# mhnazeri/PMoE

Hardware: AMD Instinct MI355X
Metric: samples/sec fwd+bwd, 256x256 RGB 4-expert PMoE (higher is better)
Workload: dtype bf16; 1 GPU; 4-expert MoE (PMoE experts), 256x256x3 x4 frames, batch 64/GPU, fwd+moe_loss+bwd, dropout 0.3; global_batch=64, parallelism=dp1

## Files before the change

pmoe_amd/csrc/conv_common.h:

```cpp
#pragma once
#include "common.h"

template <int LOG_RB, int MODE> __device__ __forceinline__ int swz_chunk(int x) {
    if (MODE == 0) return (x >> (8 - LOG_RB)) & ((1 << (LOG_RB - 4)) - 1);
    return ((x >> 1) & 1) << (LOG_RB - 5);
}

template <int LOG_RB, int MODE> __device__ __forceinline__ int lds_chunk_off(int pp, int j) {
    if (MODE == 2) return pp * 192 + (j << 4);
    return (pp << LOG_RB) + ((j ^ swz_chunk<LOG_RB, MODE>(pp)) << 4);
}

struct PatchGeom {
    int n0, n_end, e_first_img;
    int Y0, X0;
    int PH, PW, NPIX;
    int H, W, ld, coff, cmax;
    int dilate, shared;
    int step;
};

template <typename T, int LOG_RB, int NTHR, int MODE, typename TL = T>
__device__ __forceinline__ void load_halo_patch(char* patch, const T* in, const PatchGeom& g, int c0, int tid,
                                                float in_scale = 1.f) {
    constexpr int RB = 1 << LOG_RB, CPR = RB / 16, LOG_CPR = LOG_RB - 4;
    constexpr int PSTEP = NTHR / CPR;
    constexpr int VE = 16 / (int)sizeof(TL);
    constexpr bool CVT = sizeof(TL) != sizeof(T);
    constexpr int UB = CVT ? 2 : 4;
    static_assert(!CVT || (sizeof(T) == 2 && sizeof(TL) == 1), "conversion on load: bf16 -> fp8 only");
    const int pj = tid & (CPR - 1);
    int pp = tid >> LOG_CPR;
    int ix = pp % g.PW;
    const int row = pp / g.PW;
    int iy = row % g.PH, pn = row / g.PH;
    while (pp < g.NPIX) {
        v4i v[UB], v2[CVT ? UB : 1];
        int dst[UB];
#pragma unroll
        for (int u = 0; u < UB; ++u) {
            dst[u] = -1;
            if (pp < g.NPIX) {
                const int n = g.n0 + pn;
                int Y = g.Y0 + iy * g.step, X = g.X0 + ix * g.step;
                bool ok = n < g.n_end && (c0 + pj * VE) < g.cmax;
                if (g.dilate) {
                    ok = ok && Y >= 0 && X >= 0 && !((Y | X) & 1);
                    Y >>= 1; X >>= 1;
                    ok = ok && Y < g.H && X < g.W;
                } else {
                    ok = ok && (unsigned)Y < (unsigned)g.H && (unsigned)X < (unsigned)g.W;
                }
                v[u] = v4i{0, 0, 0, 0};
                if (CVT) v2[u] = v4i{0, 0, 0, 0};
                if (ok) {
                    const int nin = g.shared ? (n - g.e_first_img) : n;
                    const T* src = in + (((size_t)nin * g.H + Y) * g.W + X) * g.ld + g.coff + c0 + pj * VE;
                    v[u] = ldg16(src);
                    if (CVT) v2[u] = ldg16(src + 8);
                }
                dst[u] = pp * RB + ((pj ^ swz_chunk<LOG_RB, MODE>(pp)) << 4);
                pp += PSTEP;
                ix += PSTEP;
                while (ix >= g.PW) {
                    ix -= g.PW;
                    if (++iy == g.PH) { iy = 0; ++pn; }
                }
            }
        }
#pragma unroll
        for (int u = 0; u < UB; ++u)
            if (dst[u] >= 0) {
                if (CVT) *reinterpret_cast<v4i*>(patch + dst[u]) = cvt16_bf16_to_fp8(v[u], v2[u], in_scale);
                else *reinterpret_cast<v4i*>(patch + dst[u]) = v[u];
            }
    }
}

template <typename T, int LOG_RB, int NTHR, int MAXV>
struct PatchStage {
    static constexpr int RB = 1 << LOG_RB, CPR = RB / 16, LOG_CPR = LOG_RB - 4;
    static constexpr int PSTEP = NTHR / CPR;
    static constexpr int VE = 16 / (int)sizeof(T);
    v4i v[MAXV];

    __device__ __forceinline__ void issue(const T* in, const PatchGeom& g, int c0, int tid) {
        const int pj = tid & (CPR - 1);
        int pp = tid >> LOG_CPR;
        int ix = pp % g.PW;
        const int row = pp / g.PW;
        int iy = row % g.PH, pn = row / g.PH;
        const bool cok = (c0 + pj * VE) < g.cmax;
#pragma unroll
        for (int u = 0; u < MAXV; ++u) {
            v[u] = v4i{0, 0, 0, 0};
            if (pp < g.NPIX) {
                const int n = g.n0 + pn;
                int Y = g.Y0 + iy * g.step, X = g.X0 + ix * g.step;
                bool ok = cok && n < g.n_end;
                if (g.dilate) {
                    ok = ok && Y >= 0 && X >= 0 && !((Y | X) & 1);
                    Y >>= 1; X >>= 1;
                    ok = ok && Y < g.H && X < g.W;
                } else {
                    ok = ok && (unsigned)Y < (unsigned)g.H && (unsigned)X < (unsigned)g.W;
                }
                if (ok) {
                    const int nin = g.shared ? (n - g.e_first_img) : n;
                    v[u] = ldg16(in + (((size_t)nin * g.H + Y) * g.W + X) * g.ld + g.coff + c0 + pj * VE);
                }
            }
            pp += PSTEP;
            ix += PSTEP;
            while (ix >= g.PW) {
                ix -= g.PW;
                if (++iy == g.PH) { iy = 0; ++pn; }
            }
        }
    }

    template <int MODE> __device__ __forceinline__ void commit(char* patch, int npix, int tid) const {
        const int pj = tid & (CPR - 1);
#pragma unroll
        for (int u = 0; u < MAXV; ++u) {
            const int pp = (tid >> LOG_CPR) + u * PSTEP;
            if (pp < npix) *reinterpret_cast<v4i*>(patch + lds_chunk_off<LOG_RB, MODE>(pp, pj)) = v[u];
        }
    }
};
```

pmoe_amd/csrc/conv_dma.hip:

```cpp
#include "conv_common.h"
#include <stdlib.h>
#include "kernels.h"

namespace {

constexpr int RB = 128, LOG_RB = 7, CK = 64, BM = 256, BN = 128, NTHR = 512, VE = 8;
constexpr int WSLOT = BN * RB;
constexpr int RING = 4;
typedef __attribute__((address_space(3))) void lds_void;

__device__ __forceinline__ int cswz(int x) { return (x >> 1) & 7; }

#define VMCNT(n) asm volatile("s_waitcnt vmcnt(" #n ")" ::: "memory")

#ifdef PMOE_STAMP
#define STAMP_INIT unsigned long long st_prev = __builtin_amdgcn_s_memtime(); const unsigned long long st_r0 = __builtin_amdgcn_s_memrealtime(); unsigned st_acc[4] = {0, 0, 0, 0};
#define LAP(i) { const unsigned long long st_t = __builtin_amdgcn_s_memtime(); st_acc[i] += (unsigned)(st_t - st_prev); st_prev = st_t; }
#else
#define STAMP_INIT
#define LAP(i)
#endif

#define VMCASE(n) case n: VMCNT(n); break;
__device__ __forceinline__ void vm_wait_prod(int n) {
    switch (n) {
        VMCASE(0) VMCASE(1) VMCASE(2) VMCASE(3) VMCASE(4) VMCASE(5) VMCASE(6) VMCASE(7) VMCASE(8) VMCASE(9) VMCASE(10) VMCASE(11)
        VMCASE(12) VMCASE(13) VMCASE(14) VMCASE(15) VMCASE(16) VMCASE(17) VMCASE(18) VMCASE(19) VMCASE(20) VMCASE(21) VMCASE(22)
        VMCASE(23)
        default: VMCNT(24); break;
    }
}

template <bool MF16, bool PROD = false>
__global__ void __launch_bounds__(PROD ? NTHR + 64 : NTHR, PROD ? 1 : 2) conv3x3_dma_kernel(const ConvArgs a_in, const int pbuf_bytes) {
    ConvArgs a = a_in;
    if constexpr (PROD) {
        a.res_mode = PMOE_RES_NONE; a.res = nullptr;
        a.bias = nullptr; a.act = PMOE_ACT_NONE; a.drop_p = 0.f; a.bn = nullptr;
    }
    extern __shared__ __attribute__((aligned(16))) char smem[];
    STAMP_INIT
    const int tid = threadIdx.x, lane = tid & 63;
    const int wave = __builtin_amdgcn_readfirstlane(tid >> 6);
    const int l31 = lane & 31, h = lane >> 5;
    const int wm = wave >> 1, wn = wave & 1;

    const int nblk = a.CoutP / BN;
    const unsigned flat = xcd_remap(blockIdx.x, gridDim.x);
    const unsigned mb = flat / nblk;
    const int nb = (int)(flat % nblk);
    int t = (int)mb;
    const int px_t = t % a.tiles_x; t /= a.tiles_x;
    const int py_t = t % a.tiles_y; t /= a.tiles_y;
    const int ng = t % a.n_groups;
    const int e = t / a.n_groups;
    const int lTW = a.lTW, lTH = a.lTH;
    const int TW = 1 << lTW, TH = 1 << lTH;
    const int PW = TW + 2, PH = TH + 2;
    const int NPIX = a.TN * PH * PW;
    const int NPIECE = (NPIX + 7) >> 3;
    const int n0 = e * a.ipe + ng * a.TN, n_end = (e + 1) * a.ipe;
    const int oy0 = py_t * TH, ox0 = px_t * TW;
    const int cout0 = nb * BN;

    char* wring = smem + 2 * pbuf_bytes;

    const bf16* inb = (const bf16*)a.in + (size_t)n0 * a.H * a.W * a.in_ld + a.in_coff;
    long long in_bytes = ((long long)(n_end - n0) * a.H * a.W * a.in_ld - a.in_coff) * 2;
    if (in_bytes > 0x7ff00000ll) in_bytes = 0x7ff00000ll;
    const __amdgpu_buffer_rsrc_t rs_in = __builtin_amdgcn_make_buffer_rsrc((void*)inb, (short)0, (int)in_bytes, 0x00020000);
    const bf16* wb = (const bf16*)a.w + ((size_t)e * a.CoutP + cout0) * 9 * a.Cin;
    const __amdgpu_buffer_rsrc_t rs_w = __builtin_amdgcn_make_buffer_rsrc((void*)wb, (short)0, BN * 9 * a.Cin * 2, 0x00020000);

    constexpr int OOB = 0x7ff80000;
    if constexpr (PROD) {
        if (wave == 8) {
            int pv[48], wv[16];
#pragma unroll
            for (int i = 0; i < 48; ++i) {
                const int pp = (i << 3) + (lane >> 3);
                const int jj = lane & 7;
                const int px = pp % PW;
                const int rowq = pp / PW;
                const int prow = rowq % PH, pn = rowq / PH;
                const int Y = oy0 - 1 + prow, X = ox0 - 1 + px;
                const bool ok = pp < NPIX && n0 + pn < n_end && (unsigned)Y < (unsigned)a.H && (unsigned)X < (unsigned)a.W;
                pv[i] = ok ? ((((pn * a.H + Y) * a.W + X) * a.in_ld) << 1) + ((jj ^ cswz(px)) << 4) : OOB;
            }
#pragma unroll
            for (int i = 0; i < 16; ++i) {
                const int row = (i << 3) + (lane >> 3);
                wv[i] = ((row * 9 * a.Cin) << 1) + (((lane & 7) ^ cswz(row)) << 4);
            }
            auto req_w = [&](int slot, int tap, int c0) {
#pragma unroll
                for (int i = 0; i < 16; ++i)
                    __builtin_amdgcn_raw_ptr_buffer_load_lds(rs_w, (lds_void*)(wring + slot * WSLOT + (i << 10)), 16, wv[i],
                                                             (tap * a.Cin + c0) << 1, 0, 0);
            };
            const int nch = a.Cin / CK, TT = nch * 9;
            int after = 0;
            for (int ch = 0; ch < nch; ++ch) {
                const int c0 = ch * CK;
                const bool more = ch + 1 < nch;
#pragma unroll
                for (int tap = 0; tap < 9; ++tap) {
                    const int tt = ch * 9 + tap;
                    vm_wait_prod(after);
                    __builtin_amdgcn_s_barrier();
                    int n = 0;
                    if (tap >= 1 && tap <= 6 && more) {
#pragma unroll
                        for (int j = 0; j < 8; ++j) {
                            const int idx = (tap - 1) * 8 + j;
                            if (idx < NPIECE) {
                                __builtin_amdgcn_raw_ptr_buffer_load_lds(
                                    rs_in, (lds_void*)(smem + ((ch + 1) & 1) * pbuf_bytes + (idx << 10)), 16, pv[idx], (c0 + CK) << 1, 0, 0);
                                ++n;
                            }
                        }
                    }
                    if (tt + 2 < TT) {
                        int ntap = tap + 2, nc0 = c0;
                        if (ntap >= 9) { ntap -= 9; nc0 += CK; }
                        req_w((tt + 2) & (RING - 1), ntap, nc0);
                        n += 16;
                    }
                    after = n;
                }
            }
            return;
        }
    }
    int pvoff[6];
#pragma unroll
    for (int i = 0; i < 6; ++i) {
        const int pp = ((wave + 8 * i) << 3) + (lane >> 3);
        const int jj = lane & 7;
        int px = pp % PW;
        const int rowq = pp / PW;
        const int prow = rowq % PH, pn = rowq / PH;
        const int Y = oy0 - 1 + prow, X = ox0 - 1 + px;
        const bool ok = pp < NPIX && n0 + pn < n_end && (unsigned)Y < (unsigned)a.H && (unsigned)X < (unsigned)a.W;
        pvoff[i] = ok ? ((((pn * a.H + Y) * a.W + X) * a.in_ld) << 1) + ((jj ^ cswz(px)) << 4) : OOB;
    }
    int wvoff[2];
#pragma unroll
    for (int i = 0; i < 2; ++i) {
        const int row = ((wave + 8 * i) << 3) + (lane >> 3);
        wvoff[i] = ((row * 9 * a.Cin) << 1) + (((lane & 7) ^ cswz(row)) << 4);
    }
    const int my_pieces = (NPIECE - wave + 7) >> 3;

    auto dma_patch = [&](int i, int buf, int c0) {
        __builtin_amdgcn_raw_ptr_buffer_load_lds(rs_in, (lds_void*)(smem + buf * pbuf_bytes + ((wave + 8 * i) << 10)), 16,
                                                 pvoff[i], c0 << 1, 0, 0);
    };
    auto dma_w = [&](int slot, int tap, int c0) {
#pragma unroll
        for (int i = 0; i < 2; ++i)
            __builtin_amdgcn_raw_ptr_buffer_load_lds(rs_w, (lds_void*)(wring + slot * WSLOT + ((wave + 8 * i) << 10)), 16,
                                                     wvoff[i], (tap * a.Cin + c0) << 1, 0, 0);
    };

    int pbase[2], pcol[2];
#pragma unroll
    for (int mt = 0; mt < 2; ++mt) {
        const int p = wm * 64 + mt * 32 + l31;
        const int mx = p & (TW - 1), my = (p >> lTW) & (TH - 1), pn = p >> (lTW + lTH);
        pbase[mt] = ((pn * PH + my) * PW + mx) << LOG_RB;
        pcol[mt] = mx;
    }
    int aoff[2][4];
#pragma unroll
    for (int nt = 0; nt < 2; ++nt)
#pragma unroll
        for (int ks = 0; ks < 4; ++ks) {
            const int row = wn * 64 + nt * 32 + l31;
            aoff[nt][ks] = row * RB + (((ks * 2 + h) ^ cswz(row)) << 4);
        }

    f32x16 acc[2][2];
#pragma unroll
    for (int i = 0; i < 2; ++i)
#pragma unroll
        for (int j = 0; j < 2; ++j)
#pragma unroll
            for (int k = 0; k < 16; ++k) acc[i][j][k] = 0.f;
    f32x4 acc16[4][4];
    int pbase16[4], pcol16[4], aoff16[4][2];
    if constexpr (MF16) {
#pragma unroll
        for (int i = 0; i < 4; ++i)
#pragma unroll
            for (int j = 0; j < 4; ++j) acc16[i][j] = f32x4{0.f, 0.f, 0.f, 0.f};
#pragma unroll
        for (int mt = 0; mt < 4; ++mt) {
            const int p = wm * 64 + mt * 16 + (lane & 15);
            const int mx = p & (TW - 1), my = (p >> lTW) & (TH - 1), pn = p >> (lTW + lTH);
            pbase16[mt] = ((pn * PH + my) * PW + mx) << LOG_RB;
            pcol16[mt] = mx;
        }
#pragma unroll
        for (int nt = 0; nt < 4; ++nt)
#pragma unroll
            for (int ks = 0; ks < 2; ++ks) {
                const int row = wn * 64 + nt * 16 + (lane & 15);
                aoff16[nt][ks] = row * RB + (((ks * 4 + (lane >> 4)) ^ cswz(row)) << 4);
            }
    }

    const int nchunks = a.Cin / CK;
    const int T = nchunks * 9;

    const bool zpre_on = !PROD && (a.res_mode == PMOE_RES_DBN || a.res_mode == PMOE_RES_ADD) && !a.bias && a.act == PMOE_ACT_NONE &&
                         a.drop_p == 0.f;
    v4i zpre[8];
#pragma unroll
    for (int u = 0; u < 8; ++u) zpre[u] = v4i{0, 0, 0, 0};

#pragma unroll
    for (int i = 0; i < 6; ++i)
        if (i < my_pieces) dma_patch(i, 0, 0);
    dma_w(0, 0, 0);
    dma_w(1, 1, 0);

    for (int ch = 0; ch < nchunks; ++ch) {
        const int c0 = ch * CK;
        const char* patch = smem + (ch & 1) * pbuf_bytes;
        const bool more = ch + 1 < nchunks;
#pragma unroll
        for (int tap = 0; tap < 9; ++tap) {
            const int tt = ch * 9 + tap;
            const bool prev_piece = tap >= 2 && tap <= 7 && more && (tap - 2) < my_pieces;
            if constexpr (PROD) {
                if (tt == 0) VMCNT(0);
            } else {
                if (tt + 1 >= T) VMCNT(0);
                else if (zpre_on && !more && tap == 1) VMCNT(10);
                else if (prev_piece) VMCNT(3);
                else VMCNT(2);
            }
            __builtin_amdgcn_s_barrier();
#ifdef PMOE_STAMP
            if (tt == 0) LAP(0)
#endif
            if constexpr (!PROD) {
            if (tap >= 1 && tap <= 6 && more && (tap - 1) < my_pieces) dma_patch(tap - 1, (ch + 1) & 1, c0 + CK);
            if (tt + 2 < T) {
                int ntap = tap + 2, nc0 = c0;
                if (ntap >= 9) { ntap -= 9; nc0 += CK; }
                dma_w((tt + 2) & (RING - 1), ntap, nc0);
            }
            }
            if (tap == 0 && zpre_on && !more) {
                const int zc = tid & 15, zr = tid >> 4;
#pragma unroll
                for (int u = 0; u < 8; ++u) {
                    const int p = zr + u * 32;
                    const int mx = p & (TW - 1), my = (p >> lTW) & (TH - 1), pn = p >> (lTW + lTH);
                    const int n = n0 + pn, oy = oy0 + my, ox = ox0 + mx;
                    const bool ok = cout0 + zc * VE < a.Cout && n < n_end && oy < a.Ho && ox < a.Wo;
                    const size_t off = ok ? (((size_t)n * a.Ho + oy) * a.Wo + ox) * a.res_ld + a.res_coff + cout0 + zc * VE : (size_t)0;
                    zpre[u] = ldg16((const bf16*)a.res + off);
                }
            }
            const char* wt = wring + (tt & (RING - 1)) * WSLOT;
            const int tapoff = ((tap / 3) * PW + (tap % 3)) << LOG_RB;
            if constexpr (MF16) {
                int bsw16[4];
                const char* bp16[4];
#pragma unroll
                for (int mt = 0; mt < 4; ++mt) {
                    bp16[mt] = patch + pbase16[mt] + tapoff;
                    bsw16[mt] = cswz(pcol16[mt] + (tap % 3));
                }
#pragma unroll
                for (int ks = 0; ks < 2; ++ks) {
                    v4i af[4], bfr[4];
#pragma unroll
                    for (int nt = 0; nt < 4; ++nt) af[nt] = *reinterpret_cast<const v4i*>(wt + aoff16[nt][ks]);
#pragma unroll
                    for (int mt = 0; mt < 4; ++mt)
                        bfr[mt] = *reinterpret_cast<const v4i*>(bp16[mt] + (((ks * 4 + (lane >> 4)) ^ bsw16[mt]) << 4));
#pragma unroll
                    for (int nt = 0; nt < 4; ++nt)
#pragma unroll
                        for (int mt = 0; mt < 4; ++mt)
                            acc16[nt][mt] = __builtin_amdgcn_mfma_f32_16x16x32_bf16(__builtin_bit_cast(bf16x8, af[nt]),
                                                                                    __builtin_bit_cast(bf16x8, bfr[mt]),
                                                                                    acc16[nt][mt], 0, 0, 0);
                }
                continue;
            }
            int bsw[2];
            const char* bp[2];
#pragma unroll
            for (int mt = 0; mt < 2; ++mt) {
                bp[mt] = patch + pbase[mt] + tapoff;
                bsw[mt] = cswz(pcol[mt] + (tap % 3));
            }
#pragma unroll
            for (int ks = 0; ks < 4; ++ks) {
                v4i af[2], bfr[2];
#pragma unroll
                for (int nt = 0; nt < 2; ++nt) af[nt] = *reinterpret_cast<const v4i*>(wt + aoff[nt][ks]);
#pragma unroll
                for (int mt = 0; mt < 2; ++mt)
                    bfr[mt] = *reinterpret_cast<const v4i*>(bp[mt] + (((ks * 2 + h) ^ bsw[mt]) << 4));
#pragma unroll
                for (int nt = 0; nt < 2; ++nt)
#pragma unroll
                    for (int mt = 0; mt < 2; ++mt)
                        acc[nt][mt] = __builtin_amdgcn_mfma_f32_32x32x16_bf16(__builtin_bit_cast(bf16x8, af[nt]),
                                                                              __builtin_bit_cast(bf16x8, bfr[mt]),
                                                                              acc[nt][mt], 0, 0, 0);
            }
        }
    }

#define DMA_ZPRE zpre
#define DMA_ZPRE_ON zpre_on
#define DMA_HAS_MF16
#include "conv_dma_epilogue.inc"
#undef DMA_ZPRE
#undef DMA_ZPRE_ON
#undef DMA_HAS_MF16
}

template <bool MF16, bool NARROW = false>
__global__ void __launch_bounds__(NTHR + 4 * 64, 1) conv3x3_dma_stream_kernel(const ConvArgs a_in, const int pbuf_bytes, const int ntiles,
                                                                          const int magic_pw, const int magic_ph) {
    constexpr int NT = NARROW ? 1 : 2, WPC = 4 * NT;
    static_assert(!(NARROW && MF16), "the 64-cout tile exists on the 32x32x16 shape only");
    constexpr int BN = 64 * NT, WSLOT = BN * RB;
    STAMP_INIT
    ConvArgs a = a_in;
    a.res_mode = PMOE_RES_NONE; a.res = nullptr; a.bias = nullptr; a.act = PMOE_ACT_NONE; a.drop_p = 0.f; a.bn = nullptr;
    extern __shared__ __attribute__((aligned(16))) char smem[];
    const int tid = threadIdx.x, lane = tid & 63;
    const int wave = __builtin_amdgcn_readfirstlane(tid >> 6);
    const int l31 = lane & 31, h = lane >> 5;
    const int wm = (wave >> 1) & 3, wn = wave & 1;
    const int nblk = a.CoutP / BN;
    const int lTW = a.lTW, lTH = a.lTH;
    const int TW = 1 << lTW, TH = 1 << lTH;
    const int PW = TW + 2, PH = TH + 2;
    const int NPIX = a.TN * PH * PW;
    const int NPIECE = (NPIX + 7) >> 3;
    char* wring = smem + 2 * pbuf_bytes;
    const int nchunks = a.Cin / CK;
    const int T = nchunks * 9;
    const int G = (int)gridDim.x;
    const int b0 = (int)xcd_remap(blockIdx.x, gridDim.x);
    const int nbar_epi = a.stats ? 4 : 2;
    struct Tile { int e, n0, n_end, oy0, ox0, cout0; unsigned mb; };
    auto decode = [&](int L) {
        Tile q;
        q.mb = (unsigned)(L / nblk);
        const int nb = L % nblk;
        int t = (int)q.mb;
        const int px_t = t % a.tiles_x; t /= a.tiles_x;
        const int py_t = t % a.tiles_y; t /= a.tiles_y;
        const int ng = t % a.n_groups;
        q.e = t / a.n_groups;
        q.n0 = q.e * a.ipe + ng * a.TN; q.n_end = (q.e + 1) * a.ipe;
        q.oy0 = py_t * TH; q.ox0 = px_t * TW; q.cout0 = nb * BN;
        return q;
    };
    constexpr int OOB = 0x7ff80000;

    if (wave >= 8) {
        const int pw = wave - 8;
        auto rs_in_of = [&](const Tile& q) {
            const bf16* inb = (const bf16*)a.in + (size_t)q.e * a.ipe * a.H * a.W * a.in_ld + a.in_coff;
            return __builtin_amdgcn_make_buffer_rsrc((void*)inb, (short)0, (int)(((long long)a.ipe * a.H * a.W * a.in_ld - a.in_coff) * 2),
                                                     0x00020000);
        };
        auto rs_w_of = [&](const Tile& q) {
            const bf16* wb = (const bf16*)a.w + ((size_t)q.e * a.CoutP + q.cout0) * 9 * a.Cin;
            return __builtin_amdgcn_make_buffer_rsrc((void*)wb, (short)0, BN * 9 * a.Cin * 2, 0x00020000);
        };
        int L = b0;
        if (L >= ntiles) return;
        int gtt = 0, gch = 0;
        if (pw >= 2) {
            const int pp2 = pw - 2;
            const int lrow = lane >> 3, ljj = lane & 7;
            auto req_patch = [&](const Tile& q, const __amdgpu_buffer_rsrc_t& rs, int i, int buf, int c0, int opaque) {
                const int pp = (i << 3) + lrow + opaque;
                const int rowq = (pp * magic_pw) >> 16, px = pp - rowq * PW;
                const int pn = (rowq * magic_ph) >> 16, prow = rowq - pn * PH;
                const int n = q.n0 - q.e * a.ipe + pn, Y = q.oy0 - 1 + prow, X = q.ox0 - 1 + px;
                const bool ok = pp < NPIX && n < a.ipe && (unsigned)Y < (unsigned)a.H && (unsigned)X < (unsigned)a.W;
                const int off = ((((n * a.H + Y) * a.W + X) * a.in_ld) << 1) + ((ljj ^ cswz(px)) << 4);
                __builtin_amdgcn_raw_ptr_buffer_load_lds(rs, (lds_void*)(smem + buf * pbuf_bytes + (i << 10)), 16, ok ? off : OOB, c0 << 1, 0, 0);
            };
            Tile cur = decode(L);
            __amdgpu_buffer_rsrc_t rin = rs_in_of(cur);
            for (int i = pp2; i < NPIECE; i += 2) req_patch(cur, rin, i, 0, 0, 0);
            int after = 0;
            for (;;) {
                const bool has_next = L + G < ntiles;
                const Tile nxt = decode(has_next ? L + G : L);
                const __amdgpu_buffer_rsrc_t rin_n = rs_in_of(nxt);
                for (int ch = 0; ch < nchunks; ++ch) {
                    const int c0 = ch * CK;
                    const bool more = ch + 1 < nchunks;
                    int opaque = 0;
                    asm volatile("" : "+s"(opaque));
#pragma unroll
                    for (int tap = 0; tap < 9; ++tap) {
                        vm_wait_prod(after);
                        __builtin_amdgcn_s_barrier();
                        int n = 0;
                        if (tap >= 1 && tap <= 6 && (more || has_next)) {
#pragma unroll
                            for (int j = 0; j < 4; ++j) {
                                const int idx = (tap - 1) * 8 + 2 * j + pp2;
                                if (idx < NPIECE) {
                                    if (more) req_patch(cur, rin, idx, (gch + ch + 1) & 1, c0 + CK, opaque);
                                    else req_patch(nxt, rin_n, idx, (gch + ch + 1) & 1, 0, opaque);
                                    ++n;
                                }
                            }
                        }
                        after = n;
                    }
                }
                for (int i = 0; i < nbar_epi; ++i) __builtin_amdgcn_s_barrier();
                if (!has_next) return;
                gch += nchunks;
                L += G; cur = nxt; rin = rin_n;
            }
        }
        int wv[8];
#pragma unroll
        for (int i = 0; i < WPC; ++i) {
            const int row = ((2 * i + pw) << 3) + (lane >> 3);
            wv[i] = ((row * 9 * a.Cin) << 1) + (((lane & 7) ^ cswz(row)) << 4);
        }
        auto req_w = [&](const __amdgpu_buffer_rsrc_t& rs, int slot, int tap, int c0) {
#pragma unroll
            for (int i = 0; i < WPC; ++i)
                __builtin_amdgcn_raw_ptr_buffer_load_lds(rs, (lds_void*)(wring + slot * WSLOT + ((2 * i + pw) << 10)), 16, wv[i],
                                                         (tap * a.Cin + c0) << 1, 0, 0);
        };
        Tile cur = decode(L);
        __amdgpu_buffer_rsrc_t rw = rs_w_of(cur);
        req_w(rw, 0, 0, 0);
        req_w(rw, 1, 1, 0);
        int after = WPC;
        for (;;) {
            const bool has_next = L + G < ntiles;
            const Tile nxt = decode(has_next ? L + G : L);
            const __amdgpu_buffer_rsrc_t rw_n = rs_w_of(nxt);
            for (int ch = 0; ch < nchunks; ++ch) {
                const int c0 = ch * CK;
#pragma unroll
                for (int tap = 0; tap < 9; ++tap) {
                    const int tt = ch * 9 + tap;
                    vm_wait_prod(after);
                    __builtin_amdgcn_s_barrier();
                    int n = 0;
                    if (tt + 2 < T) {
                        int ntap = tap + 2, nc0 = c0;
                        if (ntap >= 9) { ntap -= 9; nc0 += CK; }
                        req_w(rw, (gtt + tt + 2) & (RING - 1), ntap, nc0);
                        n = WPC;
                    } else if (has_next) {
                        req_w(rw_n, (gtt + tt + 2) & (RING - 1), tt + 2 - T, 0);
                        n = WPC;
                    }
                    after = n;
                }
            }
            for (int i = 0; i < nbar_epi; ++i) __builtin_amdgcn_s_barrier();
            if (!has_next) return;
            gtt += T;
            L += G; cur = nxt; rw = rw_n;
        }
    }

    int pbase[2], pcol[2];
#pragma unroll
    for (int mt = 0; mt < 2; ++mt) {
        const int p = wm * 64 + mt * 32 + l31;
        const int mx = p & (TW - 1), my = (p >> lTW) & (TH - 1), pn = p >> (lTW + lTH);
        pbase[mt] = ((pn * PH + my) * PW + mx) << LOG_RB;
        pcol[mt] = mx;
    }
    int aoff[NT][4];
#pragma unroll
    for (int nt = 0; nt < NT; ++nt)
#pragma unroll
        for (int ks = 0; ks < 4; ++ks) {
            const int row = wn * (32 * NT) + nt * 32 + l31;
            aoff[nt][ks] = row * RB + (((ks * 2 + h) ^ cswz(row)) << 4);
        }
    int pbase16[4], pcol16[4], aoff16[4][2];
    if constexpr (MF16) {
#pragma unroll
        for (int mt = 0; mt < 4; ++mt) {
            const int p = wm * 64 + mt * 16 + (lane & 15);
            const int mx = p & (TW - 1), my = (p >> lTW) & (TH - 1), pn = p >> (lTW + lTH);
            pbase16[mt] = ((pn * PH + my) * PW + mx) << LOG_RB;
            pcol16[mt] = mx;
        }
#pragma unroll
        for (int nt = 0; nt < 4; ++nt)
#pragma unroll
            for (int ks = 0; ks < 2; ++ks) {
                const int row = wn * 64 + nt * 16 + (lane & 15);
                aoff16[nt][ks] = row * RB + (((ks * 4 + (lane >> 4)) ^ cswz(row)) << 4);
            }
    }
    int gtt = 0, gch = 0;
    for (int L = b0; L < ntiles; L += G) {
        const Tile q = decode(L);
        const int e = q.e, n0 = q.n0, n_end = q.n_end, oy0 = q.oy0, ox0 = q.ox0, cout0 = q.cout0;
        const unsigned mb = q.mb;
        f32x16 acc[NT][2];
        f32x4 acc16[4][4];
        if constexpr (MF16) {
#pragma unroll
            for (int i = 0; i < 4; ++i)
#pragma unroll
                for (int j = 0; j < 4; ++j) acc16[i][j] = f32x4{0.f, 0.f, 0.f, 0.f};
        } else {
#pragma unroll
            for (int i = 0; i < NT; ++i)
#pragma unroll
                for (int j = 0; j < 2; ++j)
#pragma unroll
                    for (int k = 0; k < 16; ++k) acc[i][j][k] = 0.f;
        }
        for (int ch = 0; ch < nchunks; ++ch) {
            const char* patch = smem + ((gch + ch) & 1) * pbuf_bytes;
#pragma unroll
            for (int tap = 0; tap < 9; ++tap) {
                const int tt = ch * 9 + tap;
                __builtin_amdgcn_s_barrier();
                const char* wt = wring + ((gtt + tt) & (RING - 1)) * WSLOT;
                const int tapoff = ((tap / 3) * PW + (tap % 3)) << LOG_RB;
                if constexpr (MF16) {
                    int bsw16[4];
                    const char* bp16[4];
#pragma unroll
                    for (int mt = 0; mt < 4; ++mt) {
                        bp16[mt] = patch + pbase16[mt] + tapoff;
                        bsw16[mt] = cswz(pcol16[mt] + (tap % 3));
                    }
#pragma unroll
                    for (int ks = 0; ks < 2; ++ks) {
                        v4i af[4], bfr[4];
#pragma unroll
                        for (int nt = 0; nt < 4; ++nt) af[nt] = *reinterpret_cast<const v4i*>(wt + aoff16[nt][ks]);
#pragma unroll
                        for (int mt = 0; mt < 4; ++mt)
                            bfr[mt] = *reinterpret_cast<const v4i*>(bp16[mt] + (((ks * 4 + (lane >> 4)) ^ bsw16[mt]) << 4));
#pragma unroll
                        for (int nt = 0; nt < 4; ++nt)
#pragma unroll
                            for (int mt = 0; mt < 4; ++mt)
                                acc16[nt][mt] = __builtin_amdgcn_mfma_f32_16x16x32_bf16(__builtin_bit_cast(bf16x8, af[nt]),
                                                                                        __builtin_bit_cast(bf16x8, bfr[mt]),
                                                                                        acc16[nt][mt], 0, 0, 0);
                    }
                } else {
                    int bsw[2];
                    const char* bp[2];
#pragma unroll
                    for (int mt = 0; mt < 2; ++mt) {
                        bp[mt] = patch + pbase[mt] + tapoff;
                        bsw[mt] = cswz(pcol[mt] + (tap % 3));
                    }
#pragma unroll
                    for (int ks = 0; ks < 4; ++ks) {
                        v4i af[NT], bfr[2];
#pragma unroll
                        for (int nt = 0; nt < NT; ++nt) af[nt] = *reinterpret_cast<const v4i*>(wt + aoff[nt][ks]);
#pragma unroll
                        for (int mt = 0; mt < 2; ++mt)
                            bfr[mt] = *reinterpret_cast<const v4i*>(bp[mt] + (((ks * 2 + h) ^ bsw[mt]) << 4));
#pragma unroll
                        for (int nt = 0; nt < NT; ++nt)
#pragma unroll
                            for (int mt = 0; mt < 2; ++mt)
                                acc[nt][mt] = __builtin_amdgcn_mfma_f32_32x32x16_bf16(__builtin_bit_cast(bf16x8, af[nt]),
                                                                                      __builtin_bit_cast(bf16x8, bfr[mt]),
                                                                                      acc[nt][mt], 0, 0, 0);
                    }
                }
            }
        }
        gtt += T; gch += nchunks;
        char* stg_lo = smem + ((gch - 1) & 1) * pbuf_bytes;
        char* stg_s0 = wring + ((gtt + 2) & (RING - 1)) * WSLOT;
        char* stg_s1 = wring + ((gtt + 3) & (RING - 1)) * WSLOT;
#define DMA_STG_ROW(p) (NT == 1 ? stg_lo + (p) * 128 : (p) < 160 ? stg_lo + (p) * 256 : (p) < 224 ? stg_s0 + ((p) - 160) * 256 : stg_s1 + ((p) - 224) * 256)
#define DMA_RED_BASE stg_lo
#define DMA_HAS_MF16
#define DMA_NT NT
#include "conv_dma_epilogue.inc"
#undef DMA_STG_ROW
#undef DMA_RED_BASE
#undef DMA_HAS_MF16
#undef DMA_NT
    }
}

__device__ __forceinline__ void vm_wait_upto(int n) {
    switch (n) {
        case 0: VMCNT(0); break; case 1: VMCNT(1); break; case 2: VMCNT(2); break; case 3: VMCNT(3); break;
        case 4: VMCNT(4); break; case 5: VMCNT(5); break; case 6: VMCNT(6); break; case 7: VMCNT(7); break;
        case 8: VMCNT(8); break; case 9: VMCNT(9); break; case 10: VMCNT(10); break; case 11: VMCNT(11); break;
        case 12: VMCNT(12); break; case 13: VMCNT(13); break; case 14: VMCNT(14); break; case 15: VMCNT(15); break;
        default: VMCNT(16); break;
    }
}

constexpr int RING3 = 3;

template <bool CLS>
__global__ void __launch_bounds__(NTHR, 2) conv3x3s2_dma_kernel(const ConvArgs a, const int pbuf_bytes) {
    extern __shared__ __attribute__((aligned(16))) char smem[];
    STAMP_INIT
    const int tid = threadIdx.x, lane = tid & 63;
    const int wave = __builtin_amdgcn_readfirstlane(tid >> 6);
    const int l31 = lane & 31, h = lane >> 5;
    const int wm = wave >> 1, wn = wave & 1;

    const int nblk = (a.CoutP + BN - 1) / BN;
    const unsigned flat = xcd_remap(blockIdx.x, gridDim.x);
    const unsigned mb = flat / nblk;
    const int nb = (int)(flat % nblk);
    int t = (int)mb;
    const int px_t = t % a.tiles_x; t /= a.tiles_x;
    const int py_t = t % a.tiles_y; t /= a.tiles_y;
    const int ng = t % a.n_groups;
    const int e = t / a.n_groups;
    const int lTW = a.lTW, lTH = a.lTH;
    const int TW = 1 << lTW, TH = 1 << lTH;
    const int PW = TW + 1, PH = TH + 1;
    const int NPIX = a.TN * PH * PW;
    const int NPIECE = (NPIX + 7) >> 3;
    const int n0 = e * a.ipe + ng * a.TN, n_end = (e + 1) * a.ipe;
    const int oy0 = py_t * TH, ox0 = px_t * TW;
    const int cout0 = nb * BN;

    char* wring = smem + 3 * pbuf_bytes;

    const bf16* inb = (const bf16*)a.in + (size_t)n0 * a.H * a.W * a.in_ld + a.in_coff;
    long long in_bytes = ((long long)(n_end - n0) * a.H * a.W * a.in_ld - a.in_coff) * 2;
    if (in_bytes > 0x7ff00000ll) in_bytes = 0x7ff00000ll;
    const __amdgpu_buffer_rsrc_t rs_in = __builtin_amdgcn_make_buffer_rsrc((void*)inb, (short)0, (int)in_bytes, 0x00020000);
    const bf16* wb = (const bf16*)a.w + ((size_t)e * a.CoutP + cout0) * 9 * a.Cin;
    const int wrows = a.CoutP - cout0 < BN ? a.CoutP - cout0 : BN;
    const __amdgpu_buffer_rsrc_t rs_w = __builtin_amdgcn_make_buffer_rsrc((void*)wb, (short)0, wrows * 9 * a.Cin * 2, 0x00020000);

    constexpr int OOB = 0x7ff80000;
    int pvoff[6];
    unsigned vbits = 0;
#pragma unroll
    for (int i = 0; i < 6; ++i) {
        const int pp = ((wave + 8 * i) << 3) + (lane >> 3);
        const int jj = lane & 7;
        const int bx = pp % PW;
        const int rowq = pp / PW;
        const int by = rowq % PH, pn = rowq / PH;
        if constexpr (CLS) {
            const int By = oy0 + by, Bx = ox0 + bx;
            const bool ok = pp < NPIX && n0 + pn < n_end && By < a.H && Bx < a.W;
            pvoff[i] = ok ? ((((pn * a.H + By) * a.W + Bx) * a.in_ld) << 1) + ((jj ^ cswz(bx)) << 4) : OOB;
        } else {
        const int By = oy0 - 1 + by, Bx = ox0 - 1 + bx;
        const bool okb = pp < NPIX && n0 + pn < n_end && By >= 0 && Bx >= 0;
        pvoff[i] = okb ? ((((pn * a.H + 2 * By) * a.W + 2 * Bx) * a.in_ld) << 1) + ((jj ^ cswz(bx)) << 4) : OOB;
        const unsigned vb = (okb && 2 * By < a.H ? 1u : 0u) | (okb && 2 * By + 1 < a.H ? 2u : 0u) |
                            (2 * Bx < a.W ? 4u : 0u) | (2 * Bx + 1 < a.W ? 8u : 0u);
        vbits |= vb << (4 * i);
        }
    }
    int wvoff[2];
#pragma unroll
    for (int i = 0; i < 2; ++i) {
        const int row = ((wave + 8 * i) << 3) + (lane >> 3);
        wvoff[i] = ((row * 9 * a.Cin) << 1) + (((lane & 7) ^ cswz(row)) << 4);
    }
    const int my_pieces = (NPIECE - wave + 7) >> 3;

    auto dma_patch = [&](int buf, int pl, int c0) {
        const int py = pl < 2, px = (pl & 1) == 0;
        const int soff = (c0 << 1) + (CLS ? 0 : (((py * a.W + px) * a.in_ld) << 1));
#pragma unroll
        for (int i = 0; i < 6; ++i)
            if (i < my_pieces) {
                const bool ok = CLS || (((vbits >> (4 * i + py)) & 1u) && ((vbits >> (4 * i + 2 + px)) & 1u));
                __builtin_amdgcn_raw_ptr_buffer_load_lds(rs_in, (lds_void*)(smem + buf * pbuf_bytes + ((wave + 8 * i) << 10)), 16,
                                                         ok ? pvoff[i] : OOB, soff, 0, 0);
            }
    };
    auto dma_w = [&](int slot, int tap, int c0) {
#pragma unroll
        for (int i = 0; i < 2; ++i)
            __builtin_amdgcn_raw_ptr_buffer_load_lds(rs_w, (lds_void*)(wring + slot * WSLOT + ((wave + 8 * i) << 10)), 16,
                                                     wvoff[i], (tap * a.Cin + c0) << 1, 0, 0);
    };
    auto tap_of = [&](int pl, int tp, int& ktap, int& oy, int& ox) {
        if constexpr (CLS) {
            oy = a.kw == 2 ? (tp >> 1) : tp; ox = a.kw == 2 ? (tp & 1) : 0;
            ktap = tp == 0 ? a.tapmap[0] : tp == 1 ? a.tapmap[1] : tp == 2 ? a.tapmap[2] : a.tapmap[3];
            return;
        }
        const int py = pl < 2, px = (pl & 1) == 0;
        const int iy = px ? (tp >> 1) : tp, ix = px ? (tp & 1) : 0;
        const int ky = py ? 2 * iy : 1, kx = px ? 2 * ix : 1;
        ktap = ky * 3 + kx;
        oy = ky != 0; ox = kx != 0;
    };
    auto ntaps = [&](int pl) { return CLS ? a.kh * a.kw : pl == 0 ? 4 : pl == 3 ? 1 : 2; };

    int pbase[2], pcol[2];
#pragma unroll
    for (int mt = 0; mt < 2; ++mt) {
        const int p = wm * 64 + mt * 32 + l31;
        const int mx = p & (TW - 1), my = (p >> lTW) & (TH - 1), pn = p >> (lTW + lTH);
        pbase[mt] = ((pn * PH + my) * PW + mx) << LOG_RB;
        pcol[mt] = mx;
    }
    int aoff[2][4];
#pragma unroll
    for (int nt = 0; nt < 2; ++nt)
#pragma unroll
        for (int ks = 0; ks < 4; ++ks) {
            const int row = wn * 64 + nt * 32 + l31;
            aoff[nt][ks] = row * RB + (((ks * 2 + h) ^ cswz(row)) << 4);
        }

    f32x16 acc[2][2];
#pragma unroll
    for (int i = 0; i < 2; ++i)
#pragma unroll
        for (int j = 0; j < 2; ++j)
#pragma unroll
            for (int k = 0; k < 16; ++k) acc[i][j][k] = 0.f;

    const int nch = a.Cin / CK;
    const int T = CLS ? nch * a.kh * a.kw : nch * 9, NSTEP = CLS ? nch : nch * 4;

    int c1 = 0, p1 = 0, p2 = 0;
    int len1 = 0, len2 = 0;
    auto step_plane = [&](int s) { return CLS ? 0 : s / nch; };
    auto step_c0 = [&](int s) { return (s % nch) * CK; };
    int pl2 = 0, ch2 = 0, tp2 = 0;
    auto advance2 = [&]() {
        if (++tp2 == ntaps(pl2)) { tp2 = 0; if (++ch2 == nch) { ch2 = 0; ++pl2; } }
    };

    dma_patch(0, step_plane(0), step_c0(0));
    if (NSTEP > 1) dma_patch(1, step_plane(1), step_c0(1));
    {
        int kt, oy, ox;
        tap_of(pl2, tp2, kt, oy, ox); dma_w(0, kt, ch2 * CK); advance2();
        if (T > 1) { tap_of(pl2, tp2, kt, oy, ox); dma_w(1, kt, ch2 * CK); advance2(); c1 = 2; }
    }

    int tt = 0, wslot = 0;
    for (int s = 0, sbuf = 0; s < NSTEP; ++s, sbuf = sbuf == 2 ? 0 : sbuf + 1) {
        const int pl = step_plane(s);
        const char* patch = smem + sbuf * pbuf_bytes;
        const int nt_s = ntaps(pl);
        for (int tp = 0; tp < nt_s; ++tp, ++tt, wslot = wslot == 2 ? 0 : wslot + 1) {
            const bool patch_last = tp == 0 && s >= 2 && len1 == 1 && len2 == 1;
            vm_wait_upto(c1 + (patch_last ? 0 : p2));
            __builtin_amdgcn_s_barrier();
            int cnow = 0, pnow = 0;
            if (tt + 2 < T) {
                int kt, oy2, ox2;
                tap_of(pl2, tp2, kt, oy2, ox2);
                dma_w(wslot == 0 ? 2 : wslot - 1, kt, ch2 * CK);
                cnow = 2;
                advance2();
            }
            if (tp == 0 && s + 2 < NSTEP) {
                dma_patch(sbuf == 0 ? 2 : sbuf - 1, step_plane(s + 2), step_c0(s + 2));
                pnow = my_pieces;
            }
            c1 = cnow + pnow; p2 = p1; p1 = pnow;
            int ktap, oy, ox;
            tap_of(pl, tp, ktap, oy, ox);
            const char* wt = wring + wslot * WSLOT;
            const int tapoff = (oy * PW + ox) << LOG_RB;
            int bsw[2];
            const char* bp[2];
#pragma unroll
            for (int mt = 0; mt < 2; ++mt) {
                bp[mt] = patch + pbase[mt] + tapoff;
                bsw[mt] = cswz(pcol[mt] + ox);
            }
#pragma unroll
            for (int ks = 0; ks < 4; ++ks) {
                v4i af[2], bfr[2];
#pragma unroll
                for (int nt = 0; nt < 2; ++nt) af[nt] = *reinterpret_cast<const v4i*>(wt + aoff[nt][ks]);
#pragma unroll
                for (int mt = 0; mt < 2; ++mt)
                    bfr[mt] = *reinterpret_cast<const v4i*>(bp[mt] + (((ks * 2 + h) ^ bsw[mt]) << 4));
#pragma unroll
                for (int nt = 0; nt < 2; ++nt)
#pragma unroll
                    for (int mt = 0; mt < 2; ++mt)
                        acc[nt][mt] = __builtin_amdgcn_mfma_f32_32x32x16_bf16(__builtin_bit_cast(bf16x8, af[nt]),
                                                                              __builtin_bit_cast(bf16x8, bfr[mt]),
                                                                              acc[nt][mt], 0, 0, 0);
            }
        }
        len2 = len1; len1 = nt_s;
    }

    if constexpr (CLS) {
#define DMA_LATTICE
#include "conv_dma_epilogue.inc"
#undef DMA_LATTICE
    } else {
#include "conv_dma_epilogue.inc"
    }
}

typedef int v8i __attribute__((ext_vector_type(8)));

__global__ void __launch_bounds__(NTHR, 2) conv3x3_dma_f8_kernel(const ConvArgs a, const int pbuf_bytes) {
    extern __shared__ __attribute__((aligned(16))) char smem[];
    STAMP_INIT
    constexpr int CK8 = 128;
    const int tid = threadIdx.x, lane = tid & 63;
    const int wave = __builtin_amdgcn_readfirstlane(tid >> 6);
    const int l31 = lane & 31, h = lane >> 5;
    const int wm = wave >> 1, wn = wave & 1;

    const int nblk = a.CoutP / BN;
    const unsigned flat = xcd_remap(blockIdx.x, gridDim.x);
    const unsigned mb = flat / nblk;
    const int nb = (int)(flat % nblk);
    int t = (int)mb;
    const int px_t = t % a.tiles_x; t /= a.tiles_x;
    const int py_t = t % a.tiles_y; t /= a.tiles_y;
    const int ng = t % a.n_groups;
    const int e = t / a.n_groups;
    const int lTW = a.lTW, lTH = a.lTH;
    const int TW = 1 << lTW, TH = 1 << lTH;
    const int PW = TW + 2, PH = TH + 2;
    const int NPIX = a.TN * PH * PW;
    const int NPIECE = (NPIX + 7) >> 3;
    const int n0 = e * a.ipe + ng * a.TN, n_end = (e + 1) * a.ipe;
    const int oy0 = py_t * TH, ox0 = px_t * TW;
    const int cout0 = nb * BN;

    char* wring = smem + 2 * pbuf_bytes;

    const unsigned char* inb = (const unsigned char*)a.in + (size_t)n0 * a.H * a.W * a.in_ld + a.in_coff;
    long long in_bytes = (long long)(n_end - n0) * a.H * a.W * a.in_ld - a.in_coff;
    if (in_bytes > 0x7ff00000ll) in_bytes = 0x7ff00000ll;
    const __amdgpu_buffer_rsrc_t rs_in = __builtin_amdgcn_make_buffer_rsrc((void*)inb, (short)0, (int)in_bytes, 0x00020000);
    const unsigned char* wb = (const unsigned char*)a.w + ((size_t)e * a.CoutP + cout0) * 9 * a.Cin;
    const __amdgpu_buffer_rsrc_t rs_w = __builtin_amdgcn_make_buffer_rsrc((void*)wb, (short)0, BN * 9 * a.Cin, 0x00020000);

    constexpr int OOB = 0x7ff80000;
    int pvoff[6];
#pragma unroll
    for (int i = 0; i < 6; ++i) {
        const int pp = ((wave + 8 * i) << 3) + (lane >> 3);
        const int jj = lane & 7;
        int px = pp % PW;
        const int rowq = pp / PW;
        const int prow = rowq % PH, pn = rowq / PH;
        const int Y = oy0 - 1 + prow, X = ox0 - 1 + px;
        const bool ok = pp < NPIX && n0 + pn < n_end && (unsigned)Y < (unsigned)a.H && (unsigned)X < (unsigned)a.W;
        pvoff[i] = ok ? (((pn * a.H + Y) * a.W + X) * a.in_ld) + ((jj ^ cswz(px)) << 4) : OOB;
    }
    int wvoff[2];
#pragma unroll
    for (int i = 0; i < 2; ++i) {
        const int row = ((wave + 8 * i) << 3) + (lane >> 3);
        wvoff[i] = (row * 9 * a.Cin) + (((lane & 7) ^ cswz(row)) << 4);
    }
    const int my_pieces = (NPIECE - wave + 7) >> 3;

    auto dma_patch = [&](int i, int buf, int c0) {
        __builtin_amdgcn_raw_ptr_buffer_load_lds(rs_in, (lds_void*)(smem + buf * pbuf_bytes + ((wave + 8 * i) << 10)), 16,
                                                 pvoff[i], c0, 0, 0);
    };
    auto dma_w = [&](int slot, int tap, int c0) {
#pragma unroll
        for (int i = 0; i < 2; ++i)
            __builtin_amdgcn_raw_ptr_buffer_load_lds(rs_w, (lds_void*)(wring + slot * WSLOT + ((wave + 8 * i) << 10)), 16,
                                                     wvoff[i], tap * a.Cin + c0, 0, 0);
    };

    int pbase[2], pcol[2];
#pragma unroll
    for (int mt = 0; mt < 2; ++mt) {
        const int p = wm * 64 + mt * 32 + l31;
        const int mx = p & (TW - 1), my = (p >> lTW) & (TH - 1), pn = p >> (lTW + lTH);
        pbase[mt] = ((pn * PH + my) * PW + mx) << LOG_RB;
        pcol[mt] = mx;
    }
    int arow[2], asw[2];
#pragma unroll
    for (int nt = 0; nt < 2; ++nt) {
        const int row = wn * 64 + nt * 32 + l31;
        arow[nt] = row * RB;
        asw[nt] = cswz(row);
    }

    f32x16 acc[2][2];
#pragma unroll
    for (int i = 0; i < 2; ++i)
#pragma unroll
        for (int j = 0; j < 2; ++j)
#pragma unroll
            for (int k = 0; k < 16; ++k) acc[i][j][k] = 0.f;

    const int nchunks = a.Cin / CK8;
    const int T = nchunks * 9;

#pragma unroll
    for (int i = 0; i < 6; ++i)
        if (i < my_pieces) dma_patch(i, 0, 0);
    dma_w(0, 0, 0);
    dma_w(1, 1, 0);

    for (int ch = 0; ch < nchunks; ++ch) {
        const int c0 = ch * CK8;
        const char* patch = smem + (ch & 1) * pbuf_bytes;
        const bool more = ch + 1 < nchunks;
#pragma unroll 1
        for (int tap = 0; tap < 9; ++tap) {
            const int tt = ch * 9 + tap;
            const bool prev_piece = tap >= 2 && tap <= 7 && more && (tap - 2) < my_pieces;
            if (tt + 1 >= T) VMCNT(0);
            else if (prev_piece) VMCNT(3);
            else VMCNT(2);
            __builtin_amdgcn_s_barrier();
            if (tap >= 1 && tap <= 6 && more && (tap - 1) < my_pieces) dma_patch(tap - 1, (ch + 1) & 1, c0 + CK8);
            if (tt + 2 < T) {
                int ntap = tap + 2, nc0 = c0;
                if (ntap >= 9) { ntap -= 9; nc0 += CK8; }
                dma_w((tt + 2) & (RING - 1), ntap, nc0);
            }
            const char* wt = wring + (tt & (RING - 1)) * WSLOT;
            const int tapoff = ((tap / 3) * PW + (tap % 3)) << LOG_RB;
            int bsw[2];
            const char* bp[2];
#pragma unroll
            for (int mt = 0; mt < 2; ++mt) {
                bp[mt] = patch + pbase[mt] + tapoff;
                bsw[mt] = cswz(pcol[mt] + (tap % 3));
            }
#pragma unroll
            for (int ks = 0; ks < 2; ++ks) {
                v8i af[2], bfr[2];
#pragma unroll
                for (int nt = 0; nt < 2; ++nt) {
                    const v4i lo = *reinterpret_cast<const v4i*>(wt + arow[nt] + (((ks * 4 + 2 * h) ^ asw[nt]) << 4));
                    const v4i hi = *reinterpret_cast<const v4i*>(wt + arow[nt] + (((ks * 4 + 2 * h + 1) ^ asw[nt]) << 4));
                    af[nt] = v8i{lo[0], lo[1], lo[2], lo[3], hi[0], hi[1], hi[2], hi[3]};
                }
#pragma unroll
                for (int mt = 0; mt < 2; ++mt) {
                    const v4i lo = *reinterpret_cast<const v4i*>(bp[mt] + (((ks * 4 + 2 * h) ^ bsw[mt]) << 4));
                    const v4i hi = *reinterpret_cast<const v4i*>(bp[mt] + (((ks * 4 + 2 * h + 1) ^ bsw[mt]) << 4));
                    bfr[mt] = v8i{lo[0], lo[1], lo[2], lo[3], hi[0], hi[1], hi[2], hi[3]};
                }
#pragma unroll
                for (int nt = 0; nt < 2; ++nt)
#pragma unroll
                    for (int mt = 0; mt < 2; ++mt)
                        acc[nt][mt] = __builtin_amdgcn_mfma_scale_f32_32x32x64_f8f6f4(af[nt], bfr[mt], acc[nt][mt], 0, 0, 0, 0x7f, 0, 0x7f);
            }
        }
    }

#define DMA_OSCALE
#include "conv_dma_epilogue.inc"
#undef DMA_OSCALE
}

}

static bool dma_tile(const ConvArgs& a, int halo, int ltw_max, int nbuf, int ring, int esz, ConvLaunch* l) {
    if ((long long)a.ipe * a.Ho * a.Wo < 4096) return false;
    auto p2 = [](int v) { int l = 0; while ((1 << l) < v) ++l; return l; };
    int lTW = p2(a.Wo); if (lTW > ltw_max) lTW = ltw_max;
    if (lTW < 4) return false;
    int lTH = p2(a.Ho); if (lTH > 8 - lTW) lTH = 8 - lTW;
    const int TN = BM >> (lTW + lTH);
    const int npiece = (TN * ((1 << lTH) + halo) * ((1 << lTW) + halo) + 7) / 8;
    if (npiece > 48) return false;
    const int pb = npiece * 1024;
    const size_t need = (size_t)nbuf * pb + (size_t)ring * WSLOT;
    if (need > 160 * 1024) return false;
    if ((long long)a.ipe * a.H * a.W * a.in_ld * esz >= 0x7ff00000ll) return false;
    ConvArgs& c = l->a;
    c = a;
    c.lTW = lTW; c.lTH = lTH; c.TN = TN;
    c.n_groups = (a.ipe + TN - 1) / TN;
    c.tiles_y = (a.Ho + (1 << lTH) - 1) >> lTH;
    c.tiles_x = (a.Wo + (1 << lTW) - 1) >> lTW;
    l->mblocks = (a.N / a.ipe) * c.n_groups * c.tiles_y * c.tiles_x;
    l->smem = need < (size_t)BM / 2 * BN * 4 ? (size_t)BM / 2 * BN * 4 : need;
    l->pbuf = pb;
    return true;
}

bool conv_dma_plan(const ConvArgs& a, int dtype, ConvLaunch* l) {
    const char* ev = getenv("PMOE_CONV_DMA");
    if ((ev && !atoi(ev)) || dtype != PMOE_DT_BF16 || a.w_fp8) return false;
    if (a.ks != 3 || a.kh != 3 || a.kw != 3 || a.use_tapmap || a.stride != 1 || a.pad != 1 || a.dilate || a.in_shared) return false;
    if (a.out_step != 1 || a.Ho != a.H || a.Wo != a.W) return false;
    if (a.Cin % CK || a.Cout % 8 || a.N % a.ipe) return false;
    const bool plain = a.res_mode == PMOE_RES_NONE && !a.bias && a.act == PMOE_ACT_NONE && a.drop_p == 0.f;
    const char* evn = getenv("PMOE_DMA_NARROW");
    bool narrow = !(evn && !atoi(evn)) && a.CoutP == 64 && a.Cin >= 2 * CK && plain;
    const char* evs = getenv("PMOE_DMA_STREAM");
    bool stream = !(evs && !atoi(evs)) && plain && (a.Cin <= 256 || (evs && atoi(evs) == 2));
#ifdef PMOE_STAMP
    narrow = stream = false;
#endif
    if (a.CoutP % BN && !narrow) return false;
    if (!dma_tile(a, 2, 5, 2, RING, 2, l)) return false;
    const ConvArgs& c = l->a;
    const int PW = (1 << c.lTW) + 2, PH = (1 << c.lTH) + 2;
    const int npiece = (c.TN * PH * PW + 7) / 8;
    const bool stream_ok = l->pbuf >= 160 * 256 && magic_div_exact(npiece * 8, PW, PH, &l->mpw, &l->mph) &&
                           c.TN * PH < 1024 && PW < 1024 && a.ipe < 2047;
    if (narrow && !stream_ok) return false;
    const char* evm = getenv("PMOE_DMA_MF16");
    const char* evp = getenv("PMOE_DMA_PRODUCER");
    l->kind = CONV_DMA;
    l->narrow = narrow;
    l->stream = narrow || (stream && stream_ok);
    l->producer = !l->stream && !(evp && !atoi(evp)) && plain && (a.Cin >= 256 || (evp && atoi(evp) == 2));
    l->mf16 = !narrow && (evm ? atoi(evm) != 0 : a.Cin >= 256);
    l->code = narrow ? 5067 : (l->mf16 ? 5017 : 5007) + (l->stream ? 40 : l->producer ? 20 : 0);
    return true;
}

bool conv_dma_s2_plan(const ConvArgs& a, int dtype, ConvLaunch* l) {
    const char* ev = getenv("PMOE_CONV_S2DMA");
    if ((ev && !atoi(ev)) || dtype != PMOE_DT_BF16 || a.w_fp8) return false;
    if (a.ks != 3 || a.kh != 3 || a.kw != 3 || a.use_tapmap || a.stride != 2 || a.pad != 1 || a.dilate || a.in_shared) return false;
    if (a.out_step != 1 || a.Ho != (a.H - 1) / 2 + 1 || a.Wo != (a.W - 1) / 2 + 1) return false;
    if (a.Cin % CK || a.CoutP % BN || a.Cout % 8 || a.N % a.ipe) return false;
    if (a.res_mode == PMOE_RES_DBN) return false;
    if (!dma_tile(a, 1, 4, 3, RING3, 2, l)) return false;
    l->kind = CONV_DMA_S2;
    l->code = 5207;
    return true;
}

bool conv_dma_s2cls_plan(const ConvArgs& a, int dtype, ConvLaunch* l) {
    const char* ev = getenv("PMOE_CONV_S2DMA");
    if ((ev && !atoi(ev)) || dtype != PMOE_DT_BF16 || a.w_fp8) return false;
    if (a.ks != 3 || !a.use_tapmap || a.out_step != 2 || a.stride != 1 || a.pad != 0 || a.dilate || a.in_shared) return false;
    if (a.kh < 1 || a.kh > 2 || a.kw < 1 || a.kw > 2) return false;
    const char* e64 = getenv("PMOE_S2CLS_64");
    if (a.Cin % CK || a.CoutP % ((e64 && atoi(e64)) ? 64 : BN) || a.Cout % 8 || a.N % a.ipe || a.stats || a.res_mode > PMOE_RES_ADD) return false;
    if (!dma_tile(a, 1, 4, 3, RING3, 2, l)) return false;
    l->kind = CONV_DMA_S2CLS;
    l->code = 5207;
    return true;
}

bool conv_dma_f8_plan(const ConvArgs& a, int dtype, ConvLaunch* l) {
    const char* ev = getenv("PMOE_CONV_F8DMA");
    if ((ev && !atoi(ev)) || dtype != PMOE_DT_BF16 || !a.w_fp8 || !a.in_fp8 || !a.oscale) return false;
    if (a.ks != 3 || a.kh != 3 || a.kw != 3 || a.use_tapmap || a.stride != 1 || a.pad != 1 || a.dilate || a.in_shared) return false;
    if (a.out_step != 1 || a.Ho != a.H || a.Wo != a.W || a.res_mode != PMOE_RES_NONE) return false;
    if (a.Cin % 128 || a.CoutP % BN || a.Cout % 8 || a.N % a.ipe || a.in_ld % 16 || a.in_coff % 16) return false;
    if (!dma_tile(a, 2, 5, 2, RING, 1, l)) return false;
    l->kind = CONV_DMA_F8;
    l->code = 8507;
    return true;
}

template <auto KERNEL, typename... Args> static int dma_go(dim3 grid, int nthr, size_t smem, hipStream_t st, Args... args) {
    HIP_RET((ensure_dyn_lds<KERNEL>(160 * 1024)));
    hipLaunchKernelGGL(KERNEL, grid, dim3(nthr), smem, st, args...);
    return (int)hipGetLastError();
}

int conv_dma_launch(const ConvLaunch& l, hipStream_t st) {
    const ConvArgs& a = l.a;
    const int wgs = l.mblocks * (a.CoutP / BN);
    switch (l.kind) {
    case CONV_DMA_F8: return dma_go<conv3x3_dma_f8_kernel>(dim3(wgs), NTHR, l.smem, st, a, l.pbuf);
    case CONV_DMA_S2: return dma_go<conv3x3s2_dma_kernel<false>>(dim3(wgs), NTHR, l.smem, st, a, l.pbuf);
    case CONV_DMA_S2CLS:
        return dma_go<conv3x3s2_dma_kernel<true>>(dim3(l.mblocks * ((a.CoutP + BN - 1) / BN)), NTHR, l.smem, st, a, l.pbuf);
    case CONV_DMA: break;
    default: return PMOE_ERR_ARG;
    }
    if (l.stream) {
        const int ntiles = l.narrow ? l.mblocks : wgs;
        const dim3 grid(ntiles < 256 ? ntiles : 256);
        if (l.narrow) return dma_go<conv3x3_dma_stream_kernel<false, true>>(grid, NTHR + 4 * 64, l.smem, st, a, l.pbuf, ntiles, l.mpw, l.mph);
        if (l.mf16) return dma_go<conv3x3_dma_stream_kernel<true>>(grid, NTHR + 4 * 64, l.smem, st, a, l.pbuf, ntiles, l.mpw, l.mph);
        return dma_go<conv3x3_dma_stream_kernel<false>>(grid, NTHR + 4 * 64, l.smem, st, a, l.pbuf, ntiles, l.mpw, l.mph);
    }
    if (l.producer) {
        if (l.mf16) return dma_go<conv3x3_dma_kernel<true, true>>(dim3(wgs), NTHR + 64, l.smem, st, a, l.pbuf);
        return dma_go<conv3x3_dma_kernel<false, true>>(dim3(wgs), NTHR + 64, l.smem, st, a, l.pbuf);
    }
    if (l.mf16) return dma_go<conv3x3_dma_kernel<true>>(dim3(wgs), NTHR, l.smem, st, a, l.pbuf);
    return dma_go<conv3x3_dma_kernel<false>>(dim3(wgs), NTHR, l.smem, st, a, l.pbuf);
}
```

pmoe_amd/csrc/conv_wgrad.hip:

```cpp
#include "conv_common.h"
#include <stdlib.h>
#include "kernels.h"

template <typename T> struct WgradCfg;
template <> struct WgradCfg<bf16> { static constexpr int WCO = 2, WCI = 2, WK = 2, NW = 8; };
template <> struct WgradCfg<float> { static constexpr int WCO = 1, WCI = 1, WK = 4, NW = 4; };

typedef __attribute__((address_space(3))) s16x4 lds_s16x4;

__device__ __forceinline__ s16x4 tr_read(const char* p) {
    return __builtin_amdgcn_ds_read_tr16_b64_v4i16((lds_s16x4*)(p));
}

template <typename T, int TAPS, int MAXV>
__global__ void __launch_bounds__(WgradCfg<T>::NW * 64) conv_wgrad_kernel(const WgradArgs a) {
    constexpr int NTHR = WgradCfg<T>::NW * 64;
    constexpr int LOG_RB = 7, RB = 128;
    constexpr int VE = 16 / (int)sizeof(T);
    constexpr int CKW = RB / (int)sizeof(T);
    constexpr int WCI = WgradCfg<T>::WCI, WK = WgradCfg<T>::WK;
    constexpr int KS = TAPS == 9 ? 3 : 1;
    constexpr int MAXDY = 256 * 8 / NTHR;
    extern __shared__ __attribute__((aligned(16))) char smem[];

    const int tid = threadIdx.x, lane = tid & 63, wave = tid >> 6;
    const int l31 = lane & 31, h = lane >> 5;
    constexpr int WCO = WgradCfg<T>::WCO;
    const int ci_sub = wave % WCI;
    const int co_sub = (wave / WCI) % WCO;
    const int k_sub = wave / (WCI * WCO);

    const int e = blockIdx.z;
    const int n_ci_blk = (a.Cin + CKW - 1) / CKW;
    const int npairs = n_ci_blk * ((a.Cout + CKW - 1) / CKW);
    const unsigned flat = xcd_remap(blockIdx.x, gridDim.x);
    const int nsplit = (int)(gridDim.x / npairs);
    const int pair = a.slice_fastest ? (int)(blockIdx.x / nsplit) : (int)(flat % npairs);
    const int split = a.slice_fastest ? (int)(blockIdx.x % nsplit) : (int)(flat / npairs);
    const int cob = pair / n_ci_blk, cib = pair % n_ci_blk;
    const int co0 = cob * CKW, ci0 = cib * CKW;

    const int lTW = a.lTW, lTH = a.lTH;
    const int TW = 1 << lTW, TH = 1 << lTH;
    const int S = KS == 1 ? 1 : a.stride, step = KS == 1 ? a.stride : 1;
    const int PW = (TW - 1) * S + KS, PH = (TH - 1) * S + KS;
    const int NPIX = a.TN * PH * PW;
    const int BMP = a.TN << (lTW + lTH);
    const int mbpe = a.n_groups * a.tiles_y * a.tiles_x;

    char* dyt = smem;
    constexpr int RS = 192;
    char* patch = smem + BMP * RS;

    f32x16 acc[TAPS];
#pragma unroll
    for (int t = 0; t < TAPS; ++t)
#pragma unroll
        for (int k = 0; k < 16; ++k) acc[t][k] = 0.f;

    const T* x = (const T*)a.x;
    const T* dy = (const T*)a.dy;
    const int mb_begin = split * a.mb_per_wg;
    int mb_end = mb_begin + a.mb_per_wg;
    if (mb_end > mbpe) mb_end = mbpe;

    PatchStage<T, LOG_RB, NTHR, MAXV> xs;
    v4i dyv[MAXDY];
    const int dyj = tid & 7;
    const bool dy_cok = co0 + dyj * VE < a.Cout;

    auto issue = [&](int mbi) {
        int t = mbi;
        const int px = t % a.tiles_x; t /= a.tiles_x;
        const int py = t % a.tiles_y; t /= a.tiles_y;
        const int ng = t;
        const int n0 = e * a.ipe + ng * a.TN, n_end = (e + 1) * a.ipe;
        const int oy0 = py * TH, ox0 = px * TW;
#pragma unroll
        for (int u = 0; u < MAXDY; ++u) {
            const int p = (tid >> 3) + u * (NTHR / 8);
            const int mx = p & (TW - 1), my = (p >> lTW) & (TH - 1), pn = p >> (lTW + lTH);
            const int n = n0 + pn, oy = oy0 + my, ox = ox0 + mx;
            dyv[u] = v4i{0, 0, 0, 0};
            if (p < BMP && dy_cok && n < n_end && oy < a.Ho && ox < a.Wo)
                dyv[u] = ldg16(dy + (((size_t)n * a.Ho + oy) * a.Wo + ox) * a.dy_ld + a.dy_coff + co0 + dyj * VE);
        }
        PatchGeom geo;
        geo.n0 = n0; geo.n_end = n_end; geo.e_first_img = e * a.ipe;
        geo.Y0 = oy0 * a.stride - a.pad; geo.X0 = ox0 * a.stride - a.pad; geo.PH = PH; geo.PW = PW; geo.NPIX = NPIX;
        geo.H = a.H; geo.W = a.W; geo.ld = a.x_ld; geo.coff = a.x_coff; geo.cmax = a.Cin;
        geo.dilate = 0; geo.shared = a.x_shared; geo.step = step;
        xs.issue(x, geo, ci0, tid);
    };
    auto commit = [&]() {
#pragma unroll
        for (int u = 0; u < MAXDY; ++u) {
            const int p = (tid >> 3) + u * (NTHR / 8);
            if (p < BMP) *reinterpret_cast<v4i*>(dyt + lds_chunk_off<LOG_RB, 2>(p, dyj)) = dyv[u];
        }
        xs.template commit<2>(patch, NPIX, tid);
    };

    if (mb_begin < mb_end) issue(mb_begin);
    for (int mbi = mb_begin; mbi < mb_end; ++mbi) {
        __syncthreads();
        commit();
        __syncthreads();
        if (mbi + 1 < mb_end) issue(mbi + 1);

#pragma unroll 2
        for (int kb = k_sub; kb < (BMP >> 4); kb += WK) {
            const int p0 = kb << 4;
            if constexpr (sizeof(T) == 2) {
                const int g = lane >> 4, q = (lane >> 2) & 3, pc = lane & 3;
                const int cblk = 16 * (g & 1) + 4 * pc;
                int pA[2], ppB[2];
#pragma unroll
                for (int tt = 0; tt < 2; ++tt) {
                    const int p = p0 + 8 * (g >> 1) + 4 * tt + q;
                    pA[tt] = p;
                    const int mx = p & (TW - 1), my = (p >> lTW) & (TH - 1), pn = p >> (lTW + lTH);
                    ppB[tt] = (pn * PH + my * S) * PW + mx * S;
                }
                const int ca = (co_sub * 32 + cblk) * 2, cb = (ci_sub * 32 + cblk) * 2;
                bf16x8 fa;
#pragma unroll
                for (int tt = 0; tt < 2; ++tt) {
                    const s16x4 r = tr_read(dyt + pA[tt] * RS + ca);
                    const bf16x4 rb = __builtin_bit_cast(bf16x4, r);
#pragma unroll
                    for (int i = 0; i < 4; ++i) fa[4 * tt + i] = rb[i];
                }
                const char* bB[2] = {patch + ppB[0] * RS + cb, patch + ppB[1] * RS + cb};
#pragma unroll
                for (int tap = 0; tap < TAPS; ++tap) {
                    const int tapoff = ((tap / KS) * PW + (tap % KS)) * RS;
                    bf16x8 fb;
#pragma unroll
                    for (int tt = 0; tt < 2; ++tt) {
                        const s16x4 r = tr_read(bB[tt] + tapoff);
                        const bf16x4 rb = __builtin_bit_cast(bf16x4, r);
#pragma unroll
                        for (int i = 0; i < 4; ++i) fb[4 * tt + i] = rb[i];
                    }
                    acc[tap] = __builtin_amdgcn_mfma_f32_32x32x16_bf16(fa, fb, acc[tap], 0, 0, 0);
                }
            } else {
#pragma unroll
                for (int m = 0; m < 8; ++m) {
                    const int p = p0 + 2 * m + h;
                    const int mx = p & (TW - 1), my = (p >> lTW) & (TH - 1), pn = p >> (lTW + lTH);
                    const int ppb = (pn * PH + my * S) * PW + mx * S;
                    const float av = *reinterpret_cast<const float*>(dyt + p * RS + (l31 << 2));
#pragma unroll
                    for (int tap = 0; tap < TAPS; ++tap) {
                        const int pp = ppb + (tap / KS) * PW + (tap % KS);
                        const float bv = *reinterpret_cast<const float*>(patch + pp * RS + (l31 << 2));
                        acc[tap] = __builtin_amdgcn_mfma_f32_32x32x2f32(av, bv, acc[tap], 0, 0, 0);
                    }
                }
            }
        }
    }

    constexpr int TPR = TAPS == 9 ? 3 : 1;
    constexpr int TILE_WAVES = WCO * WCI;
    float* red = reinterpret_cast<float*>(smem);
    const int tw = wave % TILE_WAVES;
    const int cin = ci0 + ci_sub * 32 + l31;
    const size_t slab = a.per_image ? (size_t)e * a.ipe + split
                                    : (size_t)split * gridDim.z + e;
    float* dst = (a.per_image || nsplit == 1) ? a.dw : a.part;
#pragma unroll
    for (int t0 = 0; t0 < TAPS; t0 += TPR) {
        __syncthreads();
        if (k_sub > 0) {
#pragma unroll
            for (int tp = 0; tp < TPR; ++tp)
#pragma unroll
                for (int r = 0; r < 16; ++r)
                    red[((((k_sub - 1) * TPR + tp) * TILE_WAVES + tw) * 16 + r) * 64 + lane] = acc[t0 + tp][r];
        }
        __syncthreads();
        if (k_sub == 0) {
#pragma unroll
            for (int tp = 0; tp < TPR; ++tp) {
                float* base = dst + ((slab * TAPS + t0 + tp) * a.CoutP) * a.CinP;
#pragma unroll
                for (int r = 0; r < 16; ++r) {
                    float v = acc[t0 + tp][r];
#pragma unroll
                    for (int k = 1; k < WK; ++k) v += red[((((k - 1) * TPR + tp) * TILE_WAVES + tw) * 16 + r) * 64 + lane];
                    const int cout = co0 + co_sub * 32 + (r & 3) + 8 * (r >> 2) + 4 * h;
                    base[(size_t)cout * a.CinP + cin] = v;
                }
            }
        }
    }
}

template <int PIN, int WCI = 2, bool PAIRS = false, int REQ = 0>
__global__ void __launch_bounds__(512) conv_wgrad_dma_kernel(const WgradArgs a, const int magic_pw, const int magic_ph) {
    constexpr int TAPS = 9, RS = 128, CKW = 64;
    static_assert(!PAIRS || WCI == 1, "tap pairs: the narrow wave layout only");
    static_assert(REQ == 0 || (WCI == 2 && !PAIRS && PIN == 1), "precomputed requests: the 2 x 2 x 2 wave layout only");
    constexpr int WCO = 2, WK = 8 / (WCI * WCO);
    typedef __attribute__((address_space(3))) void lds_void;
    extern __shared__ __attribute__((aligned(16))) char smem[];

    const int tid = threadIdx.x, lane = tid & 63;
    const int wave = __builtin_amdgcn_readfirstlane(tid >> 6);
    const int l31 = lane & 31, h = lane >> 5;
    const int ci_sub = wave % WCI, co_sub = (wave / WCI) % WCO, k_sub = wave / (WCI * WCO);

    const int e = blockIdx.z;
    const int n_ci_blk = (a.Cin + CKW - 1) / CKW;
    const int npairs = n_ci_blk * ((a.Cout + CKW - 1) / CKW);
    const unsigned flat = xcd_remap(blockIdx.x, gridDim.x);
    const int nsplit = (int)(gridDim.x / npairs);
    const int pair = (int)(flat % npairs), split = (int)(flat / npairs);
    const int cob = pair / n_ci_blk, cib = pair % n_ci_blk;
    const int co0 = cob * CKW, ci0 = cib * CKW;

    const int lTW = a.lTW, lTH = a.lTH;
    const int TW = 1 << lTW, TH = 1 << lTH;
    const int PW = TW + 2, PH = TH + 2;
    const int NPIX = a.TN * PH * PW;
    const int NPIECE = (NPIX + 7) >> 3;
    const int BMP = a.TN << (lTW + lTH);
    const int XB = NPIECE << 10;
    const int pair_bytes = (BMP << 7) + XB;
    const int my_pieces = (NPIECE - wave + 7) >> 3;

    f32x16 acc[TAPS];
#pragma unroll
    for (int t = 0; t < TAPS; ++t)
#pragma unroll
        for (int k = 0; k < 16; ++k) acc[t][k] = 0.f;

    const int mbpe = a.n_groups * a.tiles_y * a.tiles_x;
    const int mb_begin = split * a.mb_per_wg;
    int mb_end = mb_begin + a.mb_per_wg;
    if (mb_end > mbpe) mb_end = mbpe;

    const bf16* xb = (const bf16*)a.x + (a.x_shared ? (size_t)0 : (size_t)e * a.ipe * a.H * a.W * a.x_ld) + a.x_coff + ci0;
    const bf16* dyb = (const bf16*)a.dy + (size_t)e * a.ipe * a.Ho * a.Wo * a.dy_ld + a.dy_coff + co0;
    const __amdgpu_buffer_rsrc_t rs_x = __builtin_amdgcn_make_buffer_rsrc(
        (void*)xb, (short)0, (int)(((long long)a.ipe * a.H * a.W * a.x_ld - a.x_coff - ci0) * 2), 0x00020000);
    const __amdgpu_buffer_rsrc_t rs_dy = __builtin_amdgcn_make_buffer_rsrc(
        (void*)dyb, (short)0, (int)(((long long)a.ipe * a.Ho * a.Wo * a.dy_ld - a.dy_coff - co0) * 2), 0x00020000);
    constexpr int OOB = 0x7ff80000;

    auto issue = [&](int mbi, int buf) {
        int t = mbi;
        const int px_t = t % a.tiles_x; t /= a.tiles_x;
        const int py_t = t % a.tiles_y; t /= a.tiles_y;
        const int n0 = t * a.TN;
        const int oy0 = py_t * TH, ox0 = px_t * TW;
        char* base = smem + buf * pair_bytes;
#pragma unroll
        for (int i = 0; i < 4; ++i) {
            const int p = ((wave + 8 * i) << 3) + (lane >> 3);
            const int mx = p & (TW - 1), my = (p >> lTW) & (TH - 1), pn = p >> (lTW + lTH);
            const int n = n0 + pn, oy = oy0 + my, ox = ox0 + mx;
            const int j = (lane & 7) ^ (((p >> 1) & 1) << 2);
            const bool ok = n < a.ipe && oy < a.Ho && ox < a.Wo && co0 + j * 8 < a.Cout;
            const int voff = ok ? ((((n * a.Ho + oy) * a.Wo + ox) * a.dy_ld) << 1) + (j << 4) : OOB;
            __builtin_amdgcn_raw_ptr_buffer_load_lds(rs_dy, (lds_void*)(base + ((wave + 8 * i) << 10)), 16, voff, 0, 0, 0);
        }
#pragma unroll
        for (int i = 0; i < 6; ++i) {
            if (i < my_pieces) {
                const int pp = ((wave + 8 * i) << 3) + (lane >> 3);
                const int rowq = (pp * magic_pw) >> 16, px = pp - rowq * PW;
                const int pn = (rowq * magic_ph) >> 16, prow = rowq - pn * PH;
                const int n = n0 + pn, Y = oy0 - a.pad + prow, X = ox0 - a.pad + px;
                const int j = (lane & 7) ^ (((px >> 1) & 1) << 2);
                const bool ok = pp < NPIX && n < a.ipe && (unsigned)Y < (unsigned)a.H && (unsigned)X < (unsigned)a.W &&
                                ci0 + j * 8 < a.Cin;
                const int voff = ok ? ((((n * a.H + Y) * a.W + X) * a.x_ld) << 1) + (j << 4) : OOB;
                __builtin_amdgcn_raw_ptr_buffer_load_lds(rs_x, (lds_void*)(base + (BMP << 7) + ((wave + 8 * i) << 10)), 16,
                                                         voff, 0, 0, 0);
            }
        }
    };

    constexpr int GUARD = (1 << 9) | (1 << 19) | (1 << 29);
    int drel[4], dgeo[4], xrel[6], xgeo[6], xslot[6];
    struct Walk { int px, py, ng; };
    Walk nxtw{0, 0, 0};
    if constexpr (REQ >= 1) {
#pragma unroll
        for (int i = 0; i < 4; ++i) {
            const int p = ((wave + 8 * i) << 3) + (lane >> 3);
            const int mx = p & (TW - 1), my = (p >> lTW) & (TH - 1), pn = p >> (lTW + lTH);
            const int j = (lane & 7) ^ (((p >> 1) & 1) << 2);
            drel[i] = ((((pn * a.Ho + my) * a.Wo + mx) * a.dy_ld) << 1) + (j << 4);
            dgeo[i] = (co0 + j * 8 < a.Cout ? (pn << 20) | (my << 10) | mx : (511 << 20)) | GUARD;
        }
#pragma unroll
        for (int i = 0; i < 6; ++i) {
            xslot[i] = wave + 8 * (i < my_pieces ? i : my_pieces - 1);
            const int pp = (xslot[i] << 3) + (lane >> 3);
            const int rowq = (pp * magic_pw) >> 16, px = pp - rowq * PW;
            const int pn = (rowq * magic_ph) >> 16, prow = rowq - pn * PH;
            const int j = (lane & 7) ^ (((px >> 1) & 1) << 2);
            xrel[i] = ((((pn * a.H + prow) * a.W + px) * a.x_ld) << 1) + (j << 4);
            xgeo[i] = (pp < NPIX && ci0 + j * 8 < a.Cin ? (pn << 20) | (prow << 10) | px : (511 << 20)) | GUARD;
        }
        int t = mb_begin;
        nxtw.px = t % a.tiles_x; t /= a.tiles_x;
        nxtw.py = t % a.tiles_y; nxtw.ng = t / a.tiles_y;
    }
    auto imin = [](int x, int y) { return x < y ? x : y; };
    int rq_dbase = 0, rq_dkk = 0, rq_xbase = 0, rq_xlo = 0, rq_xkk = 0, rq_want = 0;
    auto req_begin = [&](bool live) {
        const int n0 = nxtw.ng * a.TN, oy0 = nxtw.py * TH, ox0 = nxtw.px * TW, Y0 = oy0 - a.pad, X0 = ox0 - a.pad;
        const int nmax = imin(a.ipe - n0, 511) - 1;
        rq_dbase = (((n0 * a.Ho + oy0) * a.Wo + ox0) * a.dy_ld) << 1;
        rq_dkk = (((nmax << 20) | ((imin(TH, a.Ho - oy0) - 1) << 10) | (imin(TW, a.Wo - ox0) - 1)) | GUARD) + GUARD;
        rq_xbase = (((n0 * a.H + Y0) * a.W + X0) * a.x_ld) << 1;
        rq_xlo = ((Y0 < 0 ? -Y0 : 0) << 10) | (X0 < 0 ? -X0 : 0);
        rq_xkk = (((nmax << 20) | ((imin(PH, a.H - Y0) - 1) << 10) | (imin(PW, a.W - X0) - 1)) | GUARD) + GUARD;
        rq_want = live ? GUARD : -1;
        if (++nxtw.px == a.tiles_x) { nxtw.px = 0; if (++nxtw.py == a.tiles_y) { nxtw.py = 0; ++nxtw.ng; } }
    };
    auto req_dy = [&](int i, int buf) {
        const bool ok = ((rq_dkk - dgeo[i]) & GUARD) == rq_want;
        __builtin_amdgcn_raw_ptr_buffer_load_lds(rs_dy, (lds_void*)(smem + buf * pair_bytes + ((wave + 8 * i) << 10)), 16,
                                                 ok ? rq_dbase + drel[i] : OOB, 0, 0, 0);
    };
    auto req_x = [&](int i, int buf) {
        const bool ok = ((xgeo[i] - rq_xlo) & (rq_xkk - xgeo[i]) & GUARD) == rq_want;
        __builtin_amdgcn_raw_ptr_buffer_load_lds(rs_x, (lds_void*)(smem + buf * pair_bytes + (BMP << 7) + (xslot[i] << 10)), 16,
                                                 ok ? rq_xbase + xrel[i] : OOB, 0, 0, 0);
    };
    auto req_all = [&](int buf, bool live) {
        req_begin(live);
#pragma unroll
        for (int i = 0; i < 4; ++i) req_dy(i, buf);
#pragma unroll
        for (int i = 0; i < 6; ++i) req_x(i, buf);
    };

    const int g = lane >> 4, q = (lane >> 2) & 3, pc = lane & 3;
    const int ca_sw = (((co_sub * 4 + (g & 1) * 2 + (pc >> 1)) ^ (((q >> 1) & 1) << 2)) << 4) + 8 * (pc & 1);
    int cb_sw[3];
#pragma unroll
    for (int kx = 0; kx < 3; ++kx)
        cb_sw[kx] = (((ci_sub * 4 + (g & 1) * 2 + (pc >> 1)) ^ ((((q + kx) >> 1) & 1) << 2)) << 4) + 8 * (pc & 1);

    int pairoff[5];
    if constexpr (PAIRS) {
#pragma unroll
        for (int i = 0; i < 5; ++i) {
            const int tl = 2 * i + (g & 1) > 8 ? 8 : 2 * i + (g & 1);
            const int kx = tl % 3;
            pairoff[i] = ((tl / 3) * PW + kx) * RS + ((((pc >> 1)) ^ ((((q + kx) >> 1) & 1) << 2)) << 4) + 8 * (pc & 1);
        }
    }

    if constexpr (REQ >= 1) req_all(0, mb_begin < mb_end);
    else if (mb_begin < mb_end) issue(mb_begin, 0);
    for (int mbi = mb_begin; mbi < mb_end; ++mbi) {
        const int buf = (mbi - mb_begin) & 1;
        asm volatile("s_waitcnt vmcnt(0) lgkmcnt(0)" ::: "memory");
        __builtin_amdgcn_s_barrier();
        if constexpr (REQ == 1) req_all(buf ^ 1, mbi + 1 < mb_end);
        else if constexpr (REQ == 2) req_begin(mbi + 1 < mb_end);
        else if (mbi + 1 < mb_end) issue(mbi + 1, buf ^ 1);
        const char* dyt = smem + buf * pair_bytes;
        const char* patch = dyt + (BMP << 7);
        auto frag_addr = [&](int kb, int* pA, int* ppB) {
            const int p0 = kb << 4;
#pragma unroll
            for (int tt = 0; tt < 2; ++tt) {
                const int p = p0 + 8 * (g >> 1) + 4 * tt + q;
                pA[tt] = p;
                const int mx = p & (TW - 1), my = (p >> lTW) & (TH - 1), pn = p >> (lTW + lTH);
                ppB[tt] = (pn * PH + my) * PW + mx;
            }
        };
        auto read_a = [&](const int* pA) {
            bf16x8 fa;
#pragma unroll
            for (int tt = 0; tt < 2; ++tt) {
                const s16x4 r = tr_read(dyt + pA[tt] * RS + ca_sw);
                const bf16x4 rb = __builtin_bit_cast(bf16x4, r);
#pragma unroll
                for (int i = 0; i < 4; ++i) fa[4 * tt + i] = rb[i];
            }
            return fa;
        };
        auto read_b = [&](const int* ppB, int tap) {
            const int tapoff = ((tap / 3) * PW + (tap % 3)) * RS;
            bf16x8 fb;
#pragma unroll
            for (int tt = 0; tt < 2; ++tt) {
                const s16x4 r = tr_read(patch + ppB[tt] * RS + tapoff + cb_sw[tap % 3]);
                const bf16x4 rb = __builtin_bit_cast(bf16x4, r);
#pragma unroll
                for (int i = 0; i < 4; ++i) fb[4 * tt + i] = rb[i];
            }
            return fb;
        };
#pragma unroll(REQ == 2 ? 8 : 2)
        for (int kb = k_sub; kb < (BMP >> 4); kb += WK) {
            if constexpr (REQ == 2) {
                const int it = (kb - k_sub) / WK;
                if (it < 4) req_dy(it, buf ^ 1);
                if (it < 2) { req_x(2 * it, buf ^ 1); req_x(2 * it + 1, buf ^ 1); }
                else if (it < 4) req_x(it + 2, buf ^ 1);
            }
            int pA[2], ppB[2];
            frag_addr(kb, pA, ppB);
            if (PIN >= 2) {
                bf16x8 fa = PIN == 2 ? read_a(pA) : __builtin_bit_cast(bf16x8, v4i{kb, lane, kb, lane});
                bf16x8 fb = PIN == 2 ? read_b(ppB, 0) : __builtin_bit_cast(bf16x8, v4i{lane, kb, lane, kb});
#pragma unroll
                for (int tap = 0; tap < TAPS; ++tap) acc[tap] = __builtin_amdgcn_mfma_f32_32x32x16_bf16(fa, fb, acc[tap], 0, 0, 0);
                continue;
            }
            if constexpr (PAIRS) {
                const bf16x8 fa = read_a(pA);
                auto read_pair = [&](int i) {
                    bf16x8 fb;
#pragma unroll
                    for (int tt = 0; tt < 2; ++tt) {
                        const s16x4 r = tr_read(patch + ppB[tt] * RS + pairoff[i]);
                        const bf16x4 rb = __builtin_bit_cast(bf16x4, r);
#pragma unroll
                        for (int j = 0; j < 4; ++j) fb[4 * tt + j] = rb[j];
                    }
                    return fb;
                };
                bf16x8 fbp[2];
                fbp[0] = read_pair(0);
#pragma unroll
                for (int i = 0; i < 5; ++i) {
                    if (i + 1 < 5) fbp[(i + 1) & 1] = read_pair(i + 1);
                    __builtin_amdgcn_sched_barrier(0);
                    acc[i] = __builtin_amdgcn_mfma_f32_32x32x16_bf16(fa, fbp[i & 1], acc[i], 0, 0, 0);
                    __builtin_amdgcn_sched_barrier(0);
                }
                continue;
            }
            const bf16x8 fa = read_a(pA);
            bf16x8 fbq[2];
            fbq[0] = read_b(ppB, 0);
#pragma unroll
            for (int tap = 0; tap < TAPS; ++tap) {
                if (tap + 1 < TAPS) fbq[(tap + 1) & 1] = read_b(ppB, tap + 1);
                if (PIN == 1) __builtin_amdgcn_sched_barrier(0);
                acc[tap] = __builtin_amdgcn_mfma_f32_32x32x16_bf16(fa, fbq[tap & 1], acc[tap], 0, 0, 0);
                if (PIN == 1) __builtin_amdgcn_sched_barrier(0);
            }
        }
    }

    constexpr int TPR = 3, TILE_WAVES = WCO * WCI;
    float* red = reinterpret_cast<float*>(smem);
    const int tw = wave % TILE_WAVES;
    const int cin = ci0 + ci_sub * 32 + l31;
    const size_t slab = a.per_image ? (size_t)e * a.ipe + split : (size_t)split * gridDim.z + e;
    float* dst = (a.per_image || nsplit == 1) ? a.dw : a.part;
    if constexpr (PAIRS) {
#pragma unroll
        for (int i = 0; i < 5; ++i) {
            __syncthreads();
            if (k_sub > 0) {
#pragma unroll
                for (int r = 0; r < 16; ++r) red[(((k_sub - 1) * TILE_WAVES + tw) * 16 + r) * 64 + lane] = acc[i][r];
            }
            __syncthreads();
            const int tap = 2 * i + (l31 >> 4);
            if (k_sub == 0 && tap < TAPS) {
                float* base = dst + ((slab * TAPS + tap) * a.CoutP) * a.CinP;
#pragma unroll
                for (int r = 0; r < 16; ++r) {
                    float v = acc[i][r];
#pragma unroll
                    for (int k = 1; k < WK; ++k) v += red[(((k - 1) * TILE_WAVES + tw) * 16 + r) * 64 + lane];
                    const int cout = co0 + co_sub * 32 + (r & 3) + 8 * (r >> 2) + 4 * h;
                    float* row = base + (size_t)cout * a.CinP + ci0 + (l31 & 15);
                    row[0] = v;
                    for (int z = 16; ci0 + (l31 & 15) + z < a.CinP; z += 16) row[z] = 0.f;
                }
            }
        }
        return;
    }
#pragma unroll
    for (int t0 = 0; t0 < TAPS; t0 += TPR) {
        __syncthreads();
        if (k_sub > 0) {
#pragma unroll
            for (int tp = 0; tp < TPR; ++tp)
#pragma unroll
                for (int r = 0; r < 16; ++r)
                    red[((((k_sub - 1) * TPR + tp) * TILE_WAVES + tw) * 16 + r) * 64 + lane] = acc[t0 + tp][r];
        }
        __syncthreads();
        if (k_sub == 0) {
#pragma unroll
            for (int tp = 0; tp < TPR; ++tp) {
                float* base = dst + ((slab * TAPS + t0 + tp) * a.CoutP) * a.CinP;
#pragma unroll
                for (int r = 0; r < 16; ++r) {
                    float v = acc[t0 + tp][r];
#pragma unroll
                    for (int k = 1; k < WK; ++k) v += red[((((k - 1) * TPR + tp) * TILE_WAVES + tw) * 16 + r) * 64 + lane];
                    const int cout = co0 + co_sub * 32 + (r & 3) + 8 * (r >> 2) + 4 * h;
                    base[(size_t)cout * a.CinP + cin] = v;
                    if (WCI == 1 && cin + 32 < a.CinP) base[(size_t)cout * a.CinP + cin + 32] = 0.f;
                }
            }
        }
    }
}

template <int LTW, int AHEAD = 5>
__global__ void __launch_bounds__(512) conv_wgrad_dma2_kernel(const WgradArgs a, const int magic_pw, const int magic_ph) {
    constexpr int TAPS = 9, RS = 128, CKW = 64, TW = 1 << LTW, PW = TW + 2, BMP = 256;
    typedef __attribute__((address_space(3))) void lds_void;
    extern __shared__ __attribute__((aligned(16))) char smem[];
    const int tid = threadIdx.x, lane = tid & 63;
    const int wave = __builtin_amdgcn_readfirstlane(tid >> 6);
    const int l31 = lane & 31, h = lane >> 5;

    const int e = blockIdx.z;
    const int n_ci_blk = (a.Cin + CKW - 1) / CKW;
    const int npairs = n_ci_blk * ((a.Cout + CKW - 1) / CKW);
    const unsigned flat = xcd_remap(blockIdx.x, gridDim.x);
    const int nsplit = (int)(gridDim.x / npairs);
    const int pair = (int)(flat % npairs), split = (int)(flat / npairs);
    const int cob = pair / n_ci_blk, cib = pair % n_ci_blk;
    const int co0 = cob * CKW, ci0 = cib * CKW;

    const int lTH = a.lTH, TH = 1 << lTH, PH = TH + 2;
    const int NPIX = a.TN * PH * PW;
    const int NPIECE = (NPIX + 7) >> 3;
    const int XB = NPIECE << 10;
    const int pair_bytes = (BMP << 7) + XB;
    const int mbpe = a.n_groups * a.tiles_y * a.tiles_x;
    const int mb_begin = split * a.mb_per_wg;
    int mb_end = mb_begin + a.mb_per_wg;
    if (mb_end > mbpe) mb_end = mbpe;

    if (wave >= 4) {
        const int pw = wave - 4;
        const bf16* xb = (const bf16*)a.x + (a.x_shared ? (size_t)0 : (size_t)e * a.ipe * a.H * a.W * a.x_ld) + a.x_coff + ci0;
        const bf16* dyb = (const bf16*)a.dy + (size_t)e * a.ipe * a.Ho * a.Wo * a.dy_ld + a.dy_coff + co0;
        const __amdgpu_buffer_rsrc_t rs_x = __builtin_amdgcn_make_buffer_rsrc(
            (void*)xb, (short)0, (int)(((long long)a.ipe * a.H * a.W * a.x_ld - a.x_coff - ci0) * 2), 0x00020000);
        const __amdgpu_buffer_rsrc_t rs_dy = __builtin_amdgcn_make_buffer_rsrc(
            (void*)dyb, (short)0, (int)(((long long)a.ipe * a.Ho * a.Wo * a.dy_ld - a.dy_coff - co0) * 2), 0x00020000);
        constexpr int OOB = 0x7ff80000;
        constexpr int GUARD = (1 << 9) | (1 << 19) | (1 << 29);
        int drel[8], dgeo[8], xrel[12], xgeo[12];
#pragma unroll
        for (int i = 0; i < 8; ++i) {
            const int p = ((pw + 4 * i) << 3) + (lane >> 3);
            const int mx = p & (TW - 1), my = (p >> LTW) & (TH - 1), pn = p >> (LTW + lTH);
            const int j = (lane & 7) ^ (((p >> 1) & 1) << 2);
            drel[i] = ((((pn * a.Ho + my) * a.Wo + mx) * a.dy_ld) << 1) + (j << 4);
            dgeo[i] = (co0 + j * 8 < a.Cout ? (pn << 20) | (my << 10) | mx : (511 << 20)) | GUARD;
        }
        int xslot[12];
#pragma unroll
        for (int i = 0; i < 12; ++i) {
            xslot[i] = pw + 4 * i < NPIECE ? pw + 4 * i : NPIECE - 1;
            const int pp = (xslot[i] << 3) + (lane >> 3);
            const int rowq = (pp * magic_pw) >> 16, px = pp - rowq * PW;
            const int pn = (rowq * magic_ph) >> 16, prow = rowq - pn * PH;
            const int j = (lane & 7) ^ (((px >> 1) & 1) << 2);
            xrel[i] = ((((pn * a.H + prow) * a.W + px) * a.x_ld) << 1) + (j << 4);
            xgeo[i] = (pp < NPIX && ci0 + j * 8 < a.Cin ? (pn << 20) | (prow << 10) | px : (511 << 20)) | GUARD;
        }
        int wpx, wpy, wng;
        {
            int t = mb_begin;
            wpx = t % a.tiles_x; t /= a.tiles_x;
            wpy = t % a.tiles_y; wng = t / a.tiles_y;
        }
        auto imin = [](int x, int y) { return x < y ? x : y; };
        auto req_all = [&](int buf) {
            const int n0 = wng * a.TN, oy0 = wpy * TH, ox0 = wpx * TW, Y0 = oy0 - a.pad, X0 = ox0 - a.pad;
            const int nmax = imin(a.ipe - n0, 511) - 1;
            const int dbase = (((n0 * a.Ho + oy0) * a.Wo + ox0) * a.dy_ld) << 1;
            const int dkk = (((nmax << 20) | ((imin(TH, a.Ho - oy0) - 1) << 10) | (imin(TW, a.Wo - ox0) - 1)) | GUARD) + GUARD;
            const int xbase = (((n0 * a.H + Y0) * a.W + X0) * a.x_ld) << 1;
            const int xlo = ((Y0 < 0 ? -Y0 : 0) << 10) | (X0 < 0 ? -X0 : 0);
            const int xkk = (((nmax << 20) | ((imin(PH, a.H - Y0) - 1) << 10) | (imin(PW, a.W - X0) - 1)) | GUARD) + GUARD;
            char* base = smem + buf * pair_bytes;
#pragma unroll
            for (int i = 0; i < 8; ++i) {
                const bool ok = ((dkk - dgeo[i]) & GUARD) == GUARD;
                __builtin_amdgcn_raw_ptr_buffer_load_lds(rs_dy, (lds_void*)(base + ((pw + 4 * i) << 10)), 16, ok ? dbase + drel[i] : OOB,
                                                         0, 0, 0);
            }
#pragma unroll
            for (int i = 0; i < 12; ++i) {
                const bool ok = ((xgeo[i] - xlo) & (xkk - xgeo[i]) & GUARD) == GUARD;
                __builtin_amdgcn_raw_ptr_buffer_load_lds(rs_x, (lds_void*)(base + (BMP << 7) + (xslot[i] << 10)), 16,
                                                         ok ? xbase + xrel[i] : OOB, 0, 0, 0);
            }
            if (++wpx == a.tiles_x) { wpx = 0; if (++wpy == a.tiles_y) { wpy = 0; ++wng; } }
        };
        const int nmb = mb_end - mb_begin;
#pragma unroll 1
        for (int it = 0; it <= nmb; ++it) {
            if (it > 0) {
                asm volatile("s_waitcnt vmcnt(0)" ::: "memory");
                __builtin_amdgcn_s_barrier();
            }
            if (it < nmb) req_all(it & 1);
        }
        return;
    }

    const int co_sub = wave >> 1, ci_sub = wave & 1;
    f32x16 acc[TAPS];
#pragma unroll
    for (int t = 0; t < TAPS; ++t)
#pragma unroll
        for (int k = 0; k < 16; ++k) acc[t][k] = 0.f;
    const int g = lane >> 4, q = (lane >> 2) & 3, pc = lane & 3;
    int la[2], lb[2][3];
#pragma unroll
    for (int tt = 0; tt < 2; ++tt) {
        const int pl = 8 * (g >> 1) + 4 * tt + q;
        la[tt] = pl * RS + (((co_sub * 4 + (g & 1) * 2 + (pc >> 1)) ^ (((q >> 1) & 1) << 2)) << 4) + 8 * (pc & 1);
#pragma unroll
        for (int kx = 0; kx < 3; ++kx)
            lb[tt][kx] = (pl + kx) * RS + (((ci_sub * 4 + (g & 1) * 2 + (pc >> 1)) ^ ((((q + kx) >> 1) & 1) << 2)) << 4) + 8 * (pc & 1);
    }
    constexpr int RINGB = AHEAD < 6 ? 6 : 9;
    s16x4 fa_[2][2], fb_[RINGB][2];
    auto kb_brow = [&](const char* patch, int kb) {
        const int r = LTW == 5 ? kb >> 1 : kb;
        const int colb = LTW == 5 ? (kb & 1) * 16 : 0;
        const int my = r & (TH - 1), pn = r >> lTH;
        return patch + ((pn * PH + my) * PW + colb) * RS;
    };
    auto frag8 = [](const s16x4& x, const s16x4& y) {
        const bf16x4 u = __builtin_bit_cast(bf16x4, x), v = __builtin_bit_cast(bf16x4, y);
        return bf16x8{u[0], u[1], u[2], u[3], v[0], v[1], v[2], v[3]};
    };

    for (int mbi = mb_begin; mbi < mb_end; ++mbi) {
        const int buf = (mbi - mb_begin) & 1;
        asm volatile("s_waitcnt lgkmcnt(0)" ::: "memory");
        __builtin_amdgcn_s_barrier();
        const char* dyt = smem + buf * pair_bytes;
        const char* patch = dyt + (BMP << 7);
        {
            const char* br = kb_brow(patch, 0);
#pragma unroll
            for (int tt = 0; tt < 2; ++tt) fa_[0][tt] = tr_read(dyt + la[tt]);
#pragma unroll
            for (int u = 0; u < AHEAD; ++u)
#pragma unroll
                for (int tt = 0; tt < 2; ++tt) fb_[u % RINGB][tt] = tr_read(br + ((u / 3) * PW) * RS + lb[tt][u % 3]);
        }
#pragma unroll 1
        for (int kb0 = 0; kb0 < 16; kb0 += 2) {
            const char* brow[3] = {kb_brow(patch, kb0), kb_brow(patch, kb0 + 1), kb_brow(patch, kb0 + 2 < 16 ? kb0 + 2 : 0)};
#pragma unroll
            for (int v = 0; v < 18; ++v) {
                const int kbl = v / 9, tap = v % 9;
                const bf16x8 fa = frag8(fa_[kbl][0], fa_[kbl][1]);
                acc[tap] = __builtin_amdgcn_mfma_f32_32x32x16_bf16(fa, frag8(fb_[v % RINGB][0], fb_[v % RINGB][1]), acc[tap], 0, 0, 0);
                const int w = v + AHEAD, wk = w / 9, wt = w % 9;
                if (kb0 + wk < 16) {
#pragma unroll
                    for (int tt = 0; tt < 2; ++tt)
                        fb_[w % RINGB][tt] = tr_read(brow[wk] + ((wt / 3) * PW) * RS + lb[tt][wt % 3]);
                }
                if (tap == 3 && kb0 + kbl + 1 < 16) {
#pragma unroll
                    for (int tt = 0; tt < 2; ++tt) fa_[(kbl + 1) & 1][tt] = tr_read(dyt + (kb0 + kbl + 1) * (16 * RS) + la[tt]);
                }
                __builtin_amdgcn_sched_barrier(0);
            }
        }
    }

    const int cin = ci0 + ci_sub * 32 + l31;
    const size_t slab = a.per_image ? (size_t)e * a.ipe + split : (size_t)split * gridDim.z + e;
    float* dst = (a.per_image || nsplit == 1) ? a.dw : a.part;
#pragma unroll
    for (int tap = 0; tap < TAPS; ++tap) {
        float* base = dst + ((slab * TAPS + tap) * a.CoutP) * a.CinP;
#pragma unroll
        for (int r = 0; r < 16; ++r) {
            const int cout = co0 + co_sub * 32 + (r & 3) + 8 * (r >> 2) + 4 * h;
            base[(size_t)cout * a.CinP + cin] = acc[tap][r];
        }
    }
}

struct BnBwdFuse {
    const void* z;
    const float* coef;
    const float* c1;
    const float* c2;
    int z_ld, C;
};

__global__ void __launch_bounds__(512) conv_wgrad_bnbwd_kernel(const WgradArgs a, const BnBwdFuse f) {
    constexpr int TAPS = 9, RS = 192, XRS = 32, WK = 4, TILE_WAVES = 2;
    extern __shared__ __attribute__((aligned(16))) char smem[];
    const int tid = threadIdx.x, lane = tid & 63;
    const int wave = __builtin_amdgcn_readfirstlane(tid >> 6);
    const int l31 = lane & 31, h = lane >> 5;
    const int co_sub = wave & 1, k_sub = wave >> 1;
    const int e = blockIdx.z, img = blockIdx.x;
    const int lTW = a.lTW, lTH = a.lTH;
    const int TW = 1 << lTW, TH = 1 << lTH;
    const int PW = TW + 2, PH = TH + 2, NPIX = PH * PW;
    constexpr int BMP = 256;
    char* dyt = smem;
    char* patch = smem + BMP * RS;

    f32x16 acc[5];
#pragma unroll
    for (int t = 0; t < 5; ++t)
#pragma unroll
        for (int k = 0; k < 16; ++k) acc[t][k] = 0.f;

    const size_t n_out = (size_t)e * a.ipe + img;
    const bf16* dy = (const bf16*)a.dy + n_out * a.Ho * a.Wo * a.dy_ld + a.dy_coff;
    const bf16* zz = (const bf16*)f.z + n_out * a.Ho * a.Wo * f.z_ld;
    const bf16* x = (const bf16*)a.x + (a.x_shared ? (size_t)img : n_out) * a.H * a.W * a.x_ld + a.x_coff;

    const int dyj = tid & 7;
    float A[8], Bx[8], K[8], mu[8];
#pragma unroll
    for (int k = 0; k < 8; ++k) {
        const int c = dyj * 8 + k;
        const bool ok = c < f.C;
        const size_t ec = (size_t)e * f.C + (ok ? c : 0);
        const size_t EC = (size_t)gridDim.z * f.C;
        const float sc = ok ? f.coef[2 * EC + ec] : 0.f, is = ok ? f.coef[EC + ec] : 0.f;
        mu[k] = ok ? f.coef[ec] : 0.f;
        A[k] = sc;
        Bx[k] = ok ? -sc * is * f.c2[ec] : 0.f;
        K[k] = ok ? -sc * f.c1[ec] : 0.f;
    }
    const bool dy_cok = dyj * 8 < a.Cout;
    int xiy[2], xix[2], xoff[2];
#pragma unroll
    for (int u = 0; u < 2; ++u) {
        const int it = tid + u * 512, pp = it >> 1;
        xiy[u] = pp < NPIX ? pp / PW : -100000;
        xix[u] = pp - (pp / PW) * PW;
        xoff[u] = pp * XRS + (it & 1) * 16;
    }
    const bool x_cok[2] = {0 < a.Cin, 8 < a.Cin};

    v4i dyv[4], zv[4], xv[2];
    unsigned live = 0;
    auto issue = [&](int mbi) {
        const int px = mbi % a.tiles_x, py = mbi / a.tiles_x;
        const int oy0 = py * TH, ox0 = px * TW;
        live = 0;
#pragma unroll
        for (int u = 0; u < 4; ++u) {
            const int p = (tid >> 3) + u * 64;
            const int mx = p & (TW - 1), my = p >> lTW;
            const int oy = oy0 + my, ox = ox0 + mx;
            dyv[u] = zv[u] = v4i{0, 0, 0, 0};
            if (dy_cok && oy < a.Ho && ox < a.Wo) {
                live |= 1u << u;
                const size_t pix = (size_t)oy * a.Wo + ox;
                dyv[u] = ldg16(dy + pix * a.dy_ld + dyj * 8);
                zv[u] = ldg16(zz + pix * f.z_ld + dyj * 8);
            }
        }
#pragma unroll
        for (int u = 0; u < 2; ++u) {
            const int Y = oy0 - a.pad + xiy[u], X = ox0 - a.pad + xix[u];
            xv[u] = v4i{0, 0, 0, 0};
            if (x_cok[(tid + u * 512) & 1] && (unsigned)Y < (unsigned)a.H && (unsigned)X < (unsigned)a.W)
                xv[u] = ldg16(x + ((size_t)Y * a.W + X) * a.x_ld + ((tid + u * 512) & 1) * 8);
        }
    };
    auto commit = [&]() {
#pragma unroll
        for (int u = 0; u < 4; ++u) {
            const int p = (tid >> 3) + u * 64;
            float gv[8], xz[8], o[8];
            unpack16<bf16>(dyv[u], gv);
            unpack16<bf16>(zv[u], xz);
#pragma unroll
            for (int k = 0; k < 8; ++k) o[k] = gv[k] * A[k] + ((xz[k] - mu[k]) * Bx[k] + K[k]);
            *reinterpret_cast<v4i*>(dyt + p * RS + (dyj << 4)) = (live >> u) & 1u ? pack16<bf16>(o) : v4i{0, 0, 0, 0};
        }
#pragma unroll
        for (int u = 0; u < 2; ++u)
            if (xiy[u] >= 0) *reinterpret_cast<v4i*>(patch + xoff[u]) = xv[u];
    };

    const int g = lane >> 4, q = (lane >> 2) & 3, pc = lane & 3;
    const int ca = (co_sub * 32 + 16 * (g & 1) + 4 * pc) * 2;
    int pairoff[5];
#pragma unroll
    for (int i = 0; i < 5; ++i) {
        const int tl = 2 * i + (g & 1) > 8 ? 8 : 2 * i + (g & 1);
        pairoff[i] = ((tl / 3) * PW + (tl % 3)) * XRS + 8 * pc;
    }

    const int nmb = a.tiles_y * a.tiles_x;
    issue(0);
    for (int mbi = 0; mbi < nmb; ++mbi) {
        __syncthreads();
        commit();
        __syncthreads();
        if (mbi + 1 < nmb) issue(mbi + 1);
#pragma unroll
        for (int kb = k_sub; kb < (BMP >> 4); kb += WK) {
            const int p0 = kb << 4;
            bf16x8 fa;
            const char* bB[2];
#pragma unroll
            for (int tt = 0; tt < 2; ++tt) {
                const int p = p0 + 8 * (g >> 1) + 4 * tt + q;
                const int mx = p & (TW - 1), my = p >> lTW;
                bB[tt] = patch + (my * PW + mx) * XRS;
                const bf16x4 rb = __builtin_bit_cast(bf16x4, tr_read(dyt + p * RS + ca));
#pragma unroll
                for (int i = 0; i < 4; ++i) fa[4 * tt + i] = rb[i];
            }
#pragma unroll
            for (int i = 0; i < 5; ++i) {
                bf16x8 fb;
#pragma unroll
                for (int tt = 0; tt < 2; ++tt) {
                    const bf16x4 rb = __builtin_bit_cast(bf16x4, tr_read(bB[tt] + pairoff[i]));
#pragma unroll
                    for (int j = 0; j < 4; ++j) fb[4 * tt + j] = rb[j];
                }
                acc[i] = __builtin_amdgcn_mfma_f32_32x32x16_bf16(fa, fb, acc[i], 0, 0, 0);
            }
        }
    }

    float* red = reinterpret_cast<float*>(smem);
    const size_t slab = n_out;
#pragma unroll
    for (int i = 0; i < 5; ++i) {
        __syncthreads();
        if (k_sub > 0) {
#pragma unroll
            for (int r = 0; r < 16; ++r) red[(((k_sub - 1) * TILE_WAVES + co_sub) * 16 + r) * 64 + lane] = acc[i][r];
        }
        __syncthreads();
        const int tap = 2 * i + (l31 >> 4);
        if (k_sub == 0 && tap < TAPS) {
            float* base = a.dw + ((slab * TAPS + tap) * a.CoutP) * a.CinP;
#pragma unroll
            for (int r = 0; r < 16; ++r) {
                float v = acc[i][r];
#pragma unroll
                for (int k = 1; k < WK; ++k) v += red[(((k - 1) * TILE_WAVES + co_sub) * 16 + r) * 64 + lane];
                const int cout = co_sub * 32 + (r & 3) + 8 * (r >> 2) + 4 * h;
                float* row = base + (size_t)cout * a.CinP + (l31 & 15);
                row[0] = v;
                for (int z = 16; (l31 & 15) + z < a.CinP; z += 16) row[z] = 0.f;
            }
        }
    }
}

__global__ void __launch_bounds__(256) wgrad_reduce_kernel(const float* __restrict__ part, float* __restrict__ dw,
                                                           const int nsplit, const long long total4) {
    const long long i = (long long)blockIdx.x * 256 + threadIdx.x;
    if (i >= total4) return;
    const f32x4* p = reinterpret_cast<const f32x4*>(part);
    f32x4 s = p[i];
    for (int k = 1; k < nsplit; ++k) {
        const f32x4 v = p[(long long)k * total4 + i];
        s[0] += v[0]; s[1] += v[1]; s[2] += v[2]; s[3] += v[3];
    }
    reinterpret_cast<f32x4*>(dw)[i] = s;
}

template <int TAPS>
__global__ void __launch_bounds__(256) wgrad_fold_unpack_kernel(const float* __restrict__ slabs, float* __restrict__ g,
                                                                const int nsplit, const long long slab_stride, const int cout,
                                                                const int cin, const int CoutP, const int CinP) {
    const int e = blockIdx.y;
    const long long n = (long long)cout * cin;
    const int pr = threadIdx.x & 63, tg = threadIdx.x >> 6;
    __shared__ float sm[64 * TAPS];
    for (long long i0 = (long long)blockIdx.x * 64; i0 < n; i0 += (long long)gridDim.x * 64) {
        const long long i = i0 + pr;
        if (i < n) {
            const int ci = (int)(i % cin), co = (int)(i / cin);
            for (int t = tg; t < TAPS; t += 4) {
                const float* p = slabs + (((size_t)e * TAPS + t) * CoutP + co) * CinP + ci;
                float s0 = 0.f, s1 = 0.f, s2 = 0.f, s3 = 0.f;
                int k = 0;
                for (; k + 4 <= nsplit; k += 4) {
                    s0 += p[(size_t)k * slab_stride]; s1 += p[(size_t)(k + 1) * slab_stride];
                    s2 += p[(size_t)(k + 2) * slab_stride]; s3 += p[(size_t)(k + 3) * slab_stride];
                }
                for (; k < nsplit; ++k) s0 += p[(size_t)k * slab_stride];
                sm[pr * TAPS + t] = (s0 + s1) + (s2 + s3);
            }
        }
        __syncthreads();
        const long long cnt = (n - i0 < 64 ? n - i0 : 64) * TAPS;
        float* o = g + ((size_t)e * n + i0) * TAPS;
        for (int j = threadIdx.x; j < cnt; j += 256) o[j] = sm[j];
        __syncthreads();
    }
}


static int wgrad_finish(const WgradPlan& p, hipStream_t st, bool force = false) {
    const WgradArgs& a = p.a;
    if (a.per_image || (a.defer_fold && !force)) return 0;
    const long long total = (long long)p.E * p.taps * a.CoutP * a.CinP;
    if (a.grads) {
        const float* src = p.nsplit > 1 ? a.part : a.dw;
        long long blocks = ((long long)a.cout_real * a.cin_real + 63) / 64;
        if (blocks > 4096) blocks = 4096;
        dim3 grid((unsigned)blocks, p.E);
        if (p.taps == 9)
            hipLaunchKernelGGL(wgrad_fold_unpack_kernel<9>, grid, dim3(256), 0, st, src, a.grads, p.nsplit, total, a.cout_real,
                               a.cin_real, a.CoutP, a.CinP);
        else
            hipLaunchKernelGGL(wgrad_fold_unpack_kernel<1>, grid, dim3(256), 0, st, src, a.grads, p.nsplit, total, a.cout_real,
                               a.cin_real, a.CoutP, a.CinP);
        return (int)hipGetLastError();
    }
    if (p.nsplit > 1) {
        hipLaunchKernelGGL(wgrad_reduce_kernel, dim3((unsigned)((total / 4 + 255) / 256)), dim3(256), 0, st, a.part, a.dw, p.nsplit,
                           total / 4);
        return (int)hipGetLastError();
    }
    return 0;
}

static int wgrad_p2(int v) { int l = 0; while ((1 << l) < v) ++l; return l; }

static int wgrad_bnbwd_plan(int dtype, int z_ld, WgradPlan* p) {
    WgradArgs& a = p->a;
    if (dtype != PMOE_DT_BF16 || !a.per_image || a.ks != 3 || a.stride != 1 || a.pad != 1) return PMOE_ERR_UNSUPPORTED;
    if (a.Cin > 16 || a.Cin % 8 || a.Cout > 64 || a.Cout % 8 || a.CoutP != 64 || a.CinP != 64) return PMOE_ERR_UNSUPPORTED;
    if (a.Ho != a.H || a.Wo != a.W || a.N % a.ipe || (long long)a.H * a.W < 256) return PMOE_ERR_UNSUPPORTED;
    if (z_ld % 8 || z_ld < a.Cout || a.x_ld % 8 || a.dy_ld % 8) return PMOE_ERR_ARG;
    a.lTW = wgrad_p2(a.W) > 5 ? 5 : wgrad_p2(a.W);
    a.lTH = 8 - a.lTW; a.TN = 1; a.n_groups = a.ipe;
    a.tiles_y = (a.H + (1 << a.lTH) - 1) >> a.lTH;
    a.tiles_x = (a.W + (1 << a.lTW) - 1) >> a.lTW;
    const int NPIX = ((1 << a.lTW) + 2) * ((1 << a.lTH) + 2);
    if (NPIX * 2 > 1024) return PMOE_ERR_UNSUPPORTED;
    p->kind = WGRAD_BNBWD;
    p->E = a.N / a.ipe; p->taps = 9; p->nsplit = 1; p->ws_floats = 0;
    p->grid = dim3(a.ipe, 1, p->E); p->block = dim3(512);
    p->smem = (size_t)256 * 192 + (size_t)NPIX * 32;
    if (p->smem < (size_t)3 * 2 * 4096) p->smem = (size_t)3 * 2 * 4096;
    return 7209;
}

static bool wgrad_dma_plan(int NPIX, int PW, int PH, int tiles, WgradPlan* p) {
    const WgradArgs& a = p->a;
    const char* evd = getenv("PMOE_WGRAD_DMA");
    const long long xbytes = (long long)a.ipe * a.H * a.W * a.x_ld * 2, dybytes = (long long)a.ipe * a.Ho * a.Wo * a.dy_ld * 2;
    const int npiece = (NPIX + 7) / 8;
    const size_t sm = 2 * ((size_t)256 * 128 + (size_t)npiece * 1024);
    if ((evd && !atoi(evd)) || a.ks != 3 || a.stride != 1 || a.lTW < 2 || npiece > 48 || sm > 160 * 1024 ||
        xbytes >= 0x7ff00000ll || dybytes >= 0x7ff00000ll || !magic_div_exact(npiece * 8, PW, PH, &p->mpw, &p->mph))
        return false;
    const char* evn = getenv("PMOE_WGRAD_NARROW");
    const char* ev2 = getenv("PMOE_WGRAD_V2");
    const char* evx = getenv("PMOE_WGRAD_PIPE");
    const bool narrow = a.Cin <= 32 && !(evn && !atoi(evn));
    const bool v2 = !narrow && !(ev2 && !atoi(ev2)) && !evx && (a.lTW == 4 || a.lTW == 5) && a.ipe <= 511;
    p->kind = v2 ? WGRAD_DMA2 : WGRAD_DMA;
    p->code = narrow ? 7109 : v2 ? 7309 : 7009;
    p->grid = dim3(p->nsplit * tiles, 1, p->E); p->block = dim3(512);
    p->smem = sm < 49152 ? 49152 : sm;
    const int pipe = evx ? atoi(evx) : 1;
    p->pin = 1; p->wci = narrow ? 1 : 2;
    if (v2) {
        const char* eva = getenv("PMOE_WGRAD_AHEAD");
        p->ahead = eva && atoi(eva) == 6 ? 6 : 5;
#ifdef PMOE_STAMP
    } else if (pipe == 2 || pipe == 3) {
        p->pin = pipe; p->wci = 2;
#endif
    } else if (narrow) {
        const char* evp = getenv("PMOE_WGRAD_PAIRS");
        p->pairs = a.Cin <= 16 && !(evp && !atoi(evp));
        if (p->smem < (size_t)3 * 3 * 2 * 4096) p->smem = (size_t)3 * 3 * 2 * 4096;
    } else if (pipe == 0) {
        p->pin = 0;
    } else {
        const char* evr = getenv("PMOE_WGRAD_REQ");
        const int req = a.ipe > 511 ? 0 : evr ? atoi(evr) : 1;
        p->req = req == 1 || req == 2 ? req : 0;
    }
    return true;
}

template <typename T> constexpr int wgrad_fold_waves = (WgradCfg<T>::WK - 1) * WgradCfg<T>::WCO * WgradCfg<T>::WCI;

int wgrad_select(const WgradArgs& a0, int dtype, const WgradBn& bn, WgradPlan* p) {
    *p = WgradPlan{};
    p->a = a0;
    WgradArgs& a = p->a;
    auto done = [p](int code) { return p->code = code; };
    if (bn.fused) return done(wgrad_bnbwd_plan(dtype, bn.z_ld, p));
    if (dtype != PMOE_DT_BF16 && dtype != PMOE_DT_F32) return done(PMOE_ERR_ARG);
    const int esz = p->esz = dtype == PMOE_DT_BF16 ? 2 : 4;
    const int CKW = 128 / esz, VEh = 16 / esz, NW = esz == 2 ? WgradCfg<bf16>::NW : WgradCfg<float>::NW;
    const int M1 = 48 / NW, M2 = 80 / NW;
    if (a.Cin % VEh || a.Cout % VEh || a.CinP < a.Cin || a.CoutP < a.Cout) return done(PMOE_ERR_ARG);
    if (a.CinP != (a.Cin + CKW - 1) / CKW * CKW || a.CoutP != (a.Cout + CKW - 1) / CKW * CKW) return done(PMOE_ERR_ARG);
    if ((a.ks != 1 && a.ks != 3) || (a.stride != 1 && a.stride != 2) || a.N % a.ipe) return done(PMOE_ERR_ARG);
    p->E = a.N / a.ipe; p->taps = a.ks * a.ks;
    const int lstride = a.ks == 1 ? 1 : a.stride;
    a.lTW = wgrad_p2(a.Wo) > 5 ? 5 : wgrad_p2(a.Wo);
    int lBM = 8, PW, PH, NPIX, need;
    size_t smem;
    for (;; --lBM) {
        if (lBM < 6) return done(PMOE_ERR_UNSUPPORTED);
        a.lTH = wgrad_p2(a.Ho) > lBM - a.lTW ? lBM - a.lTW : wgrad_p2(a.Ho);
        a.TN = (1 << lBM) >> (a.lTW + a.lTH);
        PW = ((1 << a.lTW) - 1) * lstride + a.ks; PH = ((1 << a.lTH) - 1) * lstride + a.ks;
        NPIX = a.TN * PH * PW;
        need = (NPIX * 8 + NW * 64 - 1) / (NW * 64);
        smem = ((size_t)(1 << lBM) + NPIX) * 192;
        if (need <= M2 && smem <= 150 * 1024) break;
    }
    a.n_groups = (a.ipe + a.TN - 1) / a.TN;
    a.tiles_y = (a.Ho + (1 << a.lTH) - 1) >> a.lTH;
    a.tiles_x = (a.Wo + (1 << a.lTW) - 1) >> a.lTW;
    const int mbpe = a.n_groups * a.tiles_y * a.tiles_x;
    const int tiles = ((a.Cout + CKW - 1) / CKW) * ((a.Cin + CKW - 1) / CKW);
    static int target = 0;
    if (!target) { const char* ev = getenv("PMOE_WGRAD_WGS"); target = ev ? atoi(ev) : 256; }
    int want = (target + tiles * p->E - 1) / (tiles * p->E);
    if (want < 1) want = 1;
    if (want > mbpe) want = mbpe;
    a.mb_per_wg = (mbpe + want - 1) / want;
    if (a.per_image) {
        if (a.TN != 1) return done(PMOE_ERR_UNSUPPORTED);
        a.mb_per_wg = a.tiles_y * a.tiles_x;
    }
    { const char* ev = getenv("PMOE_WGRAD_SLICE_FASTEST"); a.slice_fastest = ev ? atoi(ev) : 0; }
    p->nsplit = (mbpe + a.mb_per_wg - 1) / a.mb_per_wg;
    p->ws_floats = (a.per_image || p->nsplit == 1) ? 0 : (long long)p->nsplit * p->E * p->taps * a.CoutP * a.CinP;
    if (esz == 2 && lBM == 8 && wgrad_dma_plan(NPIX, PW, PH, tiles, p)) return p->code;
    p->kind = WGRAD_TILE;
    p->maxv = need <= M1 ? M1 : M2;
    p->grid = dim3(p->nsplit * tiles, 1, p->E); p->block = dim3(NW * 64);
    const size_t fold = (size_t)(esz == 2 ? wgrad_fold_waves<bf16> : wgrad_fold_waves<float>) * (p->taps == 9 ? 3 : 1) * 4096;
    p->smem = smem < fold ? fold : smem;
    return p->code = 6000 + p->taps * 100 + p->maxv;
}

template <auto KERNEL, typename... Args> static int wgrad_go(const WgradPlan& p, hipStream_t st, Args... args) {
    HIP_RET((ensure_dyn_lds<KERNEL>(160 * 1024)));
    hipLaunchKernelGGL(KERNEL, p.grid, p.block, p.smem, st, p.a, args...);
    return (int)hipGetLastError();
}

template <typename T> static int wgrad_tile_launch(const WgradPlan& p, hipStream_t st) {
    constexpr int M1 = 48 / WgradCfg<T>::NW, M2 = 80 / WgradCfg<T>::NW;
    if (p.maxv == M1) return p.taps == 9 ? wgrad_go<conv_wgrad_kernel<T, 9, M1>>(p, st) : wgrad_go<conv_wgrad_kernel<T, 1, M1>>(p, st);
    return p.taps == 9 ? wgrad_go<conv_wgrad_kernel<T, 9, M2>>(p, st) : wgrad_go<conv_wgrad_kernel<T, 1, M2>>(p, st);
}

static int wgrad_dma_launch(const WgradPlan& p, hipStream_t st) {
    switch (p.pin) {
    case 0: return wgrad_go<conv_wgrad_dma_kernel<0>>(p, st, p.mpw, p.mph);
#ifdef PMOE_STAMP
    case 2: return wgrad_go<conv_wgrad_dma_kernel<2>>(p, st, p.mpw, p.mph);
    case 3: return wgrad_go<conv_wgrad_dma_kernel<3>>(p, st, p.mpw, p.mph);
#endif
    }
    if (p.wci == 1 && p.pairs) return wgrad_go<conv_wgrad_dma_kernel<1, 1, true>>(p, st, p.mpw, p.mph);
    if (p.wci == 1) return wgrad_go<conv_wgrad_dma_kernel<1, 1>>(p, st, p.mpw, p.mph);
    if (p.req == 2) return wgrad_go<conv_wgrad_dma_kernel<1, 2, false, 2>>(p, st, p.mpw, p.mph);
    if (p.req == 1) return wgrad_go<conv_wgrad_dma_kernel<1, 2, false, 1>>(p, st, p.mpw, p.mph);
    return wgrad_go<conv_wgrad_dma_kernel<1>>(p, st, p.mpw, p.mph);
}

static int wgrad_dma2_launch(const WgradPlan& p, hipStream_t st) {
    if (p.a.lTW == 5) return p.ahead == 6 ? wgrad_go<conv_wgrad_dma2_kernel<5, 6>>(p, st, p.mpw, p.mph) : wgrad_go<conv_wgrad_dma2_kernel<5>>(p, st, p.mpw, p.mph);
    return p.ahead == 6 ? wgrad_go<conv_wgrad_dma2_kernel<4, 6>>(p, st, p.mpw, p.mph) : wgrad_go<conv_wgrad_dma2_kernel<4>>(p, st, p.mpw, p.mph);
}

static int conv_wgrad_bnbwd_launch(const WgradPlan& p, const WgradBn& bn, hipStream_t st) {
    if (!bn.z || !bn.coef || !bn.c1 || !bn.c2 || !p.a.x || !p.a.dy || !p.a.dw) return PMOE_ERR_ARG;
    return wgrad_go<conv_wgrad_bnbwd_kernel>(p, st, BnBwdFuse{bn.z, bn.coef, bn.c1, bn.c2, bn.z_ld, p.a.Cout});
}

int conv_wgrad_launch(const WgradArgs& a, int dtype, const WgradBn& bn, hipStream_t st) {
    WgradPlan p;
    if (wgrad_select(a, dtype, bn, &p) < 0) return p.code;
    if (p.ws_floats > 0 && (!a.part || a.part_floats < p.ws_floats)) return PMOE_ERR_ARG;
    const int rc = p.kind == WGRAD_BNBWD ? conv_wgrad_bnbwd_launch(p, bn, st)
                 : p.kind == WGRAD_DMA2 ? wgrad_dma2_launch(p, st)
                 : p.kind == WGRAD_DMA ? wgrad_dma_launch(p, st)
                 : p.esz == 2 ? wgrad_tile_launch<bf16>(p, st) : wgrad_tile_launch<float>(p, st);
    return rc ? rc : wgrad_finish(p, st);
}

int conv_wgrad_fold(const WgradArgs& a, int dtype, const WgradBn& bn, hipStream_t st) {
    WgradPlan p;
    if (wgrad_select(a, dtype, bn, &p) < 0) return p.code;
    if (p.ws_floats > 0 && (!a.part || a.part_floats < p.ws_floats)) return PMOE_ERR_ARG;
    return wgrad_finish(p, st, true);
}

int conv_wgrad_plan(const WgradArgs& a, int dtype, const WgradBn& bn) {
    WgradPlan p;
    return wgrad_select(a, dtype, bn, &p);
}

long long conv_wgrad_ws_floats(const WgradArgs& a, int dtype, const WgradBn& bn) {
    WgradPlan p;
    return wgrad_select(a, dtype, bn, &p) < 0 ? p.code : p.ws_floats;
}
```

Baseline: 1890 samples/s.

## Centralize LDS swizzle keys and add per-path swizzles and stride-2 wgrad patch stride

Moves the LDS XOR swizzle logic into a shared lds_layout header and gives different access paths their own keys. The MFMA16 column path now uses col&6, and stride-2 convolutions use a key that interleaves the column parity. The bf16 3x3 stride-2 weight-gradient tile kernel gets a 160-byte patch row stride instead of 192, which shrinks LDS and changes the bank mapping for the transposed reads. The aim is fewer LDS bank conflicts and a smaller LDS footprint in those kernels, at the risk of new conflicts or mismatched writer/reader swizzles.

```diff
diff --git a/pmoe_amd/csrc/conv_common.h b/pmoe_amd/csrc/conv_common.h
--- a/pmoe_amd/csrc/conv_common.h
+++ b/pmoe_amd/csrc/conv_common.h
@@ -1,5 +1,6 @@
 #pragma once
 #include "common.h"
+#include "lds_layout.h"
 
 template <int LOG_RB, int MODE> __device__ __forceinline__ int swz_chunk(int x) {
     if (MODE == 0) return (x >> (8 - LOG_RB)) & ((1 << (LOG_RB - 4)) - 1);
@@ -7,7 +8,8 @@
 }
 
 template <int LOG_RB, int MODE> __device__ __forceinline__ int lds_chunk_off(int pp, int j) {
-    if (MODE == 2) return pp * 192 + (j << 4);
+    if (MODE == 2) return lds_layout::tr_off<false>(pp, j << 4);
+    if (MODE == 3) return lds_layout::tr_off<true>(pp, j << 4);
     return (pp << LOG_RB) + ((j ^ swz_chunk<LOG_RB, MODE>(pp)) << 4);
 }
 
diff --git a/pmoe_amd/csrc/conv_dma.hip b/pmoe_amd/csrc/conv_dma.hip
--- a/pmoe_amd/csrc/conv_dma.hip
+++ b/pmoe_amd/csrc/conv_dma.hip
@@ -8,8 +8,6 @@
 constexpr int WSLOT = BN * RB;
 constexpr int RING = 4;
 typedef __attribute__((address_space(3))) void lds_void;
-
-__device__ __forceinline__ int cswz(int x) { return (x >> 1) & 7; }
 
 #define VMCNT(n) asm volatile("s_waitcnt vmcnt(" #n ")" ::: "memory")
 
@@ -85,12 +83,12 @@
                 const int prow = rowq % PH, pn = rowq / PH;
                 const int Y = oy0 - 1 + prow, X = ox0 - 1 + px;
                 const bool ok = pp < NPIX && n0 + pn < n_end && (unsigned)Y < (unsigned)a.H && (unsigned)X < (unsigned)a.W;
-                pv[i] = ok ? ((((pn * a.H + Y) * a.W + X) * a.in_ld) << 1) + ((jj ^ cswz(px)) << 4) : OOB;
+                pv[i] = ok ? ((((pn * a.H + Y) * a.W + X) * a.in_ld) << 1) + ((jj ^ lds_layout::key_col<MF16>(px)) << 4) : OOB;
             }
 #pragma unroll
             for (int i = 0; i < 16; ++i) {
                 const int row = (i << 3) + (lane >> 3);
-                wv[i] = ((row * 9 * a.Cin) << 1) + (((lane & 7) ^ cswz(row)) << 4);
+                wv[i] = ((row * 9 * a.Cin) << 1) + (((lane & 7) ^ lds_layout::key_row(row)) << 4);
             }
             auto req_w = [&](int slot, int tap, int c0) {
 #pragma unroll
@@ -142,13 +140,13 @@
         const int prow = rowq % PH, pn = rowq / PH;
         const int Y = oy0 - 1 + prow, X = ox0 - 1 + px;
         const bool ok = pp < NPIX && n0 + pn < n_end && (unsigned)Y < (unsigned)a.H && (unsigned)X < (unsigned)a.W;
-        pvoff[i] = ok ? ((((pn * a.H + Y) * a.W + X) * a.in_ld) << 1) + ((jj ^ cswz(px)) << 4) : OOB;
+        pvoff[i] = ok ? ((((pn * a.H + Y) * a.W + X) * a.in_ld) << 1) + ((jj ^ lds_layout::key_col<MF16>(px)) << 4) : OOB;
     }
     int wvoff[2];
 #pragma unroll
     for (int i = 0; i < 2; ++i) {
         const int row = ((wave + 8 * i) << 3) + (lane >> 3);
-        wvoff[i] = ((row * 9 * a.Cin) << 1) + (((lane & 7) ^ cswz(row)) << 4);
+        wvoff[i] = ((row * 9 * a.Cin) << 1) + (((lane & 7) ^ lds_layout::key_row(row)) << 4);
     }
     const int my_pieces = (NPIECE - wave + 7) >> 3;
 
@@ -177,7 +175,7 @@
 #pragma unroll
         for (int ks = 0; ks < 4; ++ks) {
             const int row = wn * 64 + nt * 32 + l31;
-            aoff[nt][ks] = row * RB + (((ks * 2 + h) ^ cswz(row)) << 4);
+            aoff[nt][ks] = row * RB + ((lds_layout::frag_chunk_mf32(ks, lane) ^ lds_layout::key_row(row)) << 4);
         }
 
     f32x16 acc[2][2];
@@ -206,7 +204,7 @@
 #pragma unroll
             for (int ks = 0; ks < 2; ++ks) {
                 const int row = wn * 64 + nt * 16 + (lane & 15);
-                aoff16[nt][ks] = row * RB + (((ks * 4 + (lane >> 4)) ^ cswz(row)) << 4);
+                aoff16[nt][ks] = row * RB + ((lds_layout::frag_chunk_mf16(ks, lane) ^ lds_layout::key_row(row)) << 4);
             }
     }
 
@@ -273,7 +271,7 @@
 #pragma unroll
                 for (int mt = 0; mt < 4; ++mt) {
                     bp16[mt] = patch + pbase16[mt] + tapoff;
-                    bsw16[mt] = cswz(pcol16[mt] + (tap % 3));
+                    bsw16[mt] = lds_layout::key_col<MF16>(pcol16[mt] + (tap % 3));
                 }
 #pragma unroll
                 for (int ks = 0; ks < 2; ++ks) {
@@ -282,7 +280,7 @@
                     for (int nt = 0; nt < 4; ++nt) af[nt] = *reinterpret_cast<const v4i*>(wt + aoff16[nt][ks]);
 #pragma unroll
                     for (int mt = 0; mt < 4; ++mt)
-                        bfr[mt] = *reinterpret_cast<const v4i*>(bp16[mt] + (((ks * 4 + (lane >> 4)) ^ bsw16[mt]) << 4));
+                        bfr[mt] = *reinterpret_cast<const v4i*>(bp16[mt] + ((lds_layout::frag_chunk_mf16(ks, lane) ^ bsw16[mt]) << 4));
 #pragma unroll
                     for (int nt = 0; nt < 4; ++nt)
 #pragma unroll
@@ -298,7 +296,7 @@
 #pragma unroll
             for (int mt = 0; mt < 2; ++mt) {
                 bp[mt] = patch + pbase[mt] + tapoff;
-                bsw[mt] = cswz(pcol[mt] + (tap % 3));
+                bsw[mt] = lds_layout::key_col<MF16>(pcol[mt] + (tap % 3));
             }
 #pragma unroll
             for (int ks = 0; ks < 4; ++ks) {
@@ -307,7 +305,7 @@
                 for (int nt = 0; nt < 2; ++nt) af[nt] = *reinterpret_cast<const v4i*>(wt + aoff[nt][ks]);
 #pragma unroll
                 for (int mt = 0; mt < 2; ++mt)
-                    bfr[mt] = *reinterpret_cast<const v4i*>(bp[mt] + (((ks * 2 + h) ^ bsw[mt]) << 4));
+                    bfr[mt] = *reinterpret_cast<const v4i*>(bp[mt] + ((lds_layout::frag_chunk_mf32(ks, lane) ^ bsw[mt]) << 4));
 #pragma unroll
                 for (int nt = 0; nt < 2; ++nt)
 #pragma unroll
@@ -393,7 +391,7 @@
                 const int pn = (rowq * magic_ph) >> 16, prow = rowq - pn * PH;
                 const int n = q.n0 - q.e * a.ipe + pn, Y = q.oy0 - 1 + prow, X = q.ox0 - 1 + px;
                 const bool ok = pp < NPIX && n < a.ipe && (unsigned)Y < (unsigned)a.H && (unsigned)X < (unsigned)a.W;
-                const int off = ((((n * a.H + Y) * a.W + X) * a.in_ld) << 1) + ((ljj ^ cswz(px)) << 4);
+                const int off = ((((n * a.H + Y) * a.W + X) * a.in_ld) << 1) + ((ljj ^ lds_layout::key_col<MF16>(px)) << 4);
                 __builtin_amdgcn_raw_ptr_buffer_load_lds(rs, (lds_void*)(smem + buf * pbuf_bytes + (i << 10)), 16, ok ? off : OOB, c0 << 1, 0, 0);
             };
             Tile cur = decode(L);
@@ -438,7 +436,7 @@
 #pragma unroll
         for (int i = 0; i < WPC; ++i) {
             const int row = ((2 * i + pw) << 3) + (lane >> 3);
-            wv[i] = ((row * 9 * a.Cin) << 1) + (((lane & 7) ^ cswz(row)) << 4);
+            wv[i] = ((row * 9 * a.Cin) << 1) + (((lane & 7) ^ lds_layout::key_row(row)) << 4);
         }
         auto req_w = [&](const __amdgpu_buffer_rsrc_t& rs, int slot, int tap, int c0) {
 #pragma unroll
@@ -496,7 +494,7 @@
 #pragma unroll
         for (int ks = 0; ks < 4; ++ks) {
             const int row = wn * (32 * NT) + nt * 32 + l31;
-            aoff[nt][ks] = row * RB + (((ks * 2 + h) ^ cswz(row)) << 4);
+            aoff[nt][ks] = row * RB + ((lds_layout::frag_chunk_mf32(ks, lane) ^ lds_layout::key_row(row)) << 4);
         }
     int pbase16[4], pcol16[4], aoff16[4][2];
     if constexpr (MF16) {
@@ -512,7 +510,7 @@
 #pragma unroll
             for (int ks = 0; ks < 2; ++ks) {
                 const int row = wn * 64 + nt * 16 + (lane & 15);
-                aoff16[nt][ks] = row * RB + (((ks * 4 + (lane >> 4)) ^ cswz(row)) << 4);
+                aoff16[nt][ks] = row * RB + ((lds_layout::frag_chunk_mf16(ks, lane) ^ lds_layout::key_row(row)) << 4);
             }
     }
     int gtt = 0, gch = 0;
@@ -549,7 +547,7 @@
 #pragma unroll
                     for (int mt = 0; mt < 4; ++mt) {
                         bp16[mt] = patch + pbase16[mt] + tapoff;
-                        bsw16[mt] = cswz(pcol16[mt] + (tap % 3));
+                        bsw16[mt] = lds_layout::key_col<MF16>(pcol16[mt] + (tap % 3));
                     }
 #pragma unroll
                     for (int ks = 0; ks < 2; ++ks) {
@@ -558,7 +556,7 @@
                         for (int nt = 0; nt < 4; ++nt) af[nt] = *reinterpret_cast<const v4i*>(wt + aoff16[nt][ks]);
 #pragma unroll
                         for (int mt = 0; mt < 4; ++mt)
-                            bfr[mt] = *reinterpret_cast<const v4i*>(bp16[mt] + (((ks * 4 + (lane >> 4)) ^ bsw16[mt]) << 4));
+                            bfr[mt] = *reinterpret_cast<const v4i*>(bp16[mt] + ((lds_layout::frag_chunk_mf16(ks, lane) ^ bsw16[mt]) << 4));
 #pragma unroll
                         for (int nt = 0; nt < 4; ++nt)
 #pragma unroll
@@ -573,7 +571,7 @@
 #pragma unroll
                     for (int mt = 0; mt < 2; ++mt) {
                         bp[mt] = patch + pbase[mt] + tapoff;
-                        bsw[mt] = cswz(pcol[mt] + (tap % 3));
+                        bsw[mt] = lds_layout::key_col<MF16>(pcol[mt] + (tap % 3));
                     }
 #pragma unroll
                     for (int ks = 0; ks < 4; ++ks) {
@@ -582,7 +580,7 @@
                         for (int nt = 0; nt < NT; ++nt) af[nt] = *reinterpret_cast<const v4i*>(wt + aoff[nt][ks]);
 #pragma unroll
                         for (int mt = 0; mt < 2; ++mt)
-                            bfr[mt] = *reinterpret_cast<const v4i*>(bp[mt] + (((ks * 2 + h) ^ bsw[mt]) << 4));
+                            bfr[mt] = *reinterpret_cast<const v4i*>(bp[mt] + ((lds_layout::frag_chunk_mf32(ks, lane) ^ bsw[mt]) << 4));
 #pragma unroll
                         for (int nt = 0; nt < NT; ++nt)
 #pragma unroll
@@ -672,11 +670,11 @@
         if constexpr (CLS) {
             const int By = oy0 + by, Bx = ox0 + bx;
             const bool ok = pp < NPIX && n0 + pn < n_end && By < a.H && Bx < a.W;
-            pvoff[i] = ok ? ((((pn * a.H + By) * a.W + Bx) * a.in_ld) << 1) + ((jj ^ cswz(bx)) << 4) : OOB;
+            pvoff[i] = ok ? ((((pn * a.H + By) * a.W + Bx) * a.in_ld) << 1) + ((jj ^ lds_layout::key_col_s2(bx)) << 4) : OOB;
         } else {
         const int By = oy0 - 1 + by, Bx = ox0 - 1 + bx;
         const bool okb = pp < NPIX && n0 + pn < n_end && By >= 0 && Bx >= 0;
-        pvoff[i] = okb ? ((((pn * a.H + 2 * By) * a.W + 2 * Bx) * a.in_ld) << 1) + ((jj ^ cswz(bx)) << 4) : OOB;
+        pvoff[i] = okb ? ((((pn * a.H + 2 * By) * a.W + 2 * Bx) * a.in_ld) << 1) + ((jj ^ lds_layout::key_col_s2(bx)) << 4) : OOB;
         const unsigned vb = (okb && 2 * By < a.H ? 1u : 0u) | (okb && 2 * By + 1 < a.H ? 2u : 0u) |
                             (2 * Bx < a.W ? 4u : 0u) | (2 * Bx + 1 < a.W ? 8u : 0u);
         vbits |= vb << (4 * i);
@@ -686,7 +684,7 @@
 #pragma unroll
     for (int i = 0; i < 2; ++i) {
         const int row = ((wave + 8 * i) << 3) + (lane >> 3);
-        wvoff[i] = ((row * 9 * a.Cin) << 1) + (((lane & 7) ^ cswz(row)) << 4);
+        wvoff[i] = ((row * 9 * a.Cin) << 1) + (((lane & 7) ^ lds_layout::key_row(row)) << 4);
     }
     const int my_pieces = (NPIECE - wave + 7) >> 3;
 
@@ -735,7 +733,7 @@
 #pragma unroll
         for (int ks = 0; ks < 4; ++ks) {
             const int row = wn * 64 + nt * 32 + l31;
-            aoff[nt][ks] = row * RB + (((ks * 2 + h) ^ cswz(row)) << 4);
+            aoff[nt][ks] = row * RB + ((lds_layout::frag_chunk_mf32(ks, lane) ^ lds_layout::key_row(row)) << 4);
         }
 
     f32x16 acc[2][2];
@@ -797,7 +795,7 @@
 #pragma unroll
             for (int mt = 0; mt < 2; ++mt) {
                 bp[mt] = patch + pbase[mt] + tapoff;
-                bsw[mt] = cswz(pcol[mt] + ox);
+                bsw[mt] = lds_layout::key_col_s2(pcol[mt] + ox);
             }
 #pragma unroll
             for (int ks = 0; ks < 4; ++ks) {
@@ -806,7 +804,7 @@
                 for (int nt = 0; nt < 2; ++nt) af[nt] = *reinterpret_cast<const v4i*>(wt + aoff[nt][ks]);
 #pragma unroll
                 for (int mt = 0; mt < 2; ++mt)
-                    bfr[mt] = *reinterpret_cast<const v4i*>(bp[mt] + (((ks * 2 + h) ^ bsw[mt]) << 4));
+                    bfr[mt] = *reinterpret_cast<const v4i*>(bp[mt] + ((lds_layout::frag_chunk_mf32(ks, lane) ^ bsw[mt]) << 4));
 #pragma unroll
                 for (int nt = 0; nt < 2; ++nt)
 #pragma unroll
@@ -877,13 +875,13 @@
         const int prow = rowq % PH, pn = rowq / PH;
         const int Y = oy0 - 1 + prow, X = ox0 - 1 + px;
         const bool ok = pp < NPIX && n0 + pn < n_end && (unsigned)Y < (unsigned)a.H && (unsigned)X < (unsigned)a.W;
-        pvoff[i] = ok ? (((pn * a.H + Y) * a.W + X) * a.in_ld) + ((jj ^ cswz(px)) << 4) : OOB;
+        pvoff[i] = ok ? (((pn * a.H + Y) * a.W + X) * a.in_ld) + ((jj ^ lds_layout::key_col<false>(px)) << 4) : OOB;
     }
     int wvoff[2];
 #pragma unroll
     for (int i = 0; i < 2; ++i) {
         const int row = ((wave + 8 * i) << 3) + (lane >> 3);
-        wvoff[i] = (row * 9 * a.Cin) + (((lane & 7) ^ cswz(row)) << 4);
+        wvoff[i] = (row * 9 * a.Cin) + (((lane & 7) ^ lds_layout::key_row(row)) << 4);
     }
     const int my_pieces = (NPIECE - wave + 7) >> 3;
 
@@ -911,7 +909,7 @@
     for (int nt = 0; nt < 2; ++nt) {
         const int row = wn * 64 + nt * 32 + l31;
         arow[nt] = row * RB;
-        asw[nt] = cswz(row);
+        asw[nt] = lds_layout::key_row(row);
     }
 
     f32x16 acc[2][2];
@@ -956,7 +954,7 @@
 #pragma unroll
             for (int mt = 0; mt < 2; ++mt) {
                 bp[mt] = patch + pbase[mt] + tapoff;
-                bsw[mt] = cswz(pcol[mt] + (tap % 3));
+                bsw[mt] = lds_layout::key_col<false>(pcol[mt] + (tap % 3));
             }
 #pragma unroll
             for (int ks = 0; ks < 2; ++ks) {
diff --git a/pmoe_amd/csrc/conv_wgrad.hip b/pmoe_amd/csrc/conv_wgrad.hip
--- a/pmoe_amd/csrc/conv_wgrad.hip
+++ b/pmoe_amd/csrc/conv_wgrad.hip
@@ -12,8 +12,9 @@
     return __builtin_amdgcn_ds_read_tr16_b64_v4i16((lds_s16x4*)(p));
 }
 
-template <typename T, int TAPS, int MAXV>
+template <typename T, int TAPS, int MAXV, bool S2 = false>
 __global__ void __launch_bounds__(WgradCfg<T>::NW * 64) conv_wgrad_kernel(const WgradArgs a) {
+    static_assert(!S2 || (sizeof(T) == 2 && TAPS == 9), "the stride-2 patch stride serves the bf16 3x3 transposed reads");
     constexpr int NTHR = WgradCfg<T>::NW * 64;
     constexpr int LOG_RB = 7, RB = 128;
     constexpr int VE = 16 / (int)sizeof(T);
@@ -49,7 +50,8 @@
     const int mbpe = a.n_groups * a.tiles_y * a.tiles_x;
 
     char* dyt = smem;
-    constexpr int RS = 192;
+    constexpr int RS = lds_layout::tr_row_b<false>();
+    constexpr int PRS = lds_layout::tr_row_b<S2>();
     char* patch = smem + BMP * RS;
 
     f32x16 acc[TAPS];
@@ -98,7 +100,7 @@
             const int p = (tid >> 3) + u * (NTHR / 8);
             if (p < BMP) *reinterpret_cast<v4i*>(dyt + lds_chunk_off<LOG_RB, 2>(p, dyj)) = dyv[u];
         }
-        xs.template commit<2>(patch, NPIX, tid);
+        xs.template commit<S2 ? 3 : 2>(patch, NPIX, tid);
     };
 
     if (mb_begin < mb_end) issue(mb_begin);
@@ -131,10 +133,10 @@
 #pragma unroll
                     for (int i = 0; i < 4; ++i) fa[4 * tt + i] = rb[i];
                 }
-                const char* bB[2] = {patch + ppB[0] * RS + cb, patch + ppB[1] * RS + cb};
+                const char* bB[2] = {patch + ppB[0] * PRS + cb, patch + ppB[1] * PRS + cb};
 #pragma unroll
                 for (int tap = 0; tap < TAPS; ++tap) {
-                    const int tapoff = ((tap / KS) * PW + (tap % KS)) * RS;
+                    const int tapoff = ((tap / KS) * PW + (tap % KS)) * PRS;
                     bf16x8 fb;
 #pragma unroll
                     for (int tt = 0; tt < 2; ++tt) {
@@ -155,7 +157,7 @@
 #pragma unroll
                     for (int tap = 0; tap < TAPS; ++tap) {
                         const int pp = ppb + (tap / KS) * PW + (tap % KS);
-                        const float bv = *reinterpret_cast<const float*>(patch + pp * RS + (l31 << 2));
+                        const float bv = *reinterpret_cast<const float*>(patch + pp * PRS + (l31 << 2));
                         acc[tap] = __builtin_amdgcn_mfma_f32_32x32x2f32(av, bv, acc[tap], 0, 0, 0);
                     }
                 }
@@ -709,7 +711,7 @@
 };
 
 __global__ void __launch_bounds__(512) conv_wgrad_bnbwd_kernel(const WgradArgs a, const BnBwdFuse f) {
-    constexpr int TAPS = 9, RS = 192, XRS = 32, WK = 4, TILE_WAVES = 2;
+    constexpr int TAPS = 9, RS = lds_layout::TR_ROW_B, XRS = 32, WK = 4, TILE_WAVES = 2;
     extern __shared__ __attribute__((aligned(16))) char smem[];
     const int tid = threadIdx.x, lane = tid & 63;
     const int wave = __builtin_amdgcn_readfirstlane(tid >> 6);
@@ -961,7 +963,7 @@
     p->kind = WGRAD_BNBWD;
     p->E = a.N / a.ipe; p->taps = 9; p->nsplit = 1; p->ws_floats = 0;
     p->grid = dim3(a.ipe, 1, p->E); p->block = dim3(512);
-    p->smem = (size_t)256 * 192 + (size_t)NPIX * 32;
+    p->smem = (size_t)256 * lds_layout::TR_ROW_B + (size_t)NPIX * 32;
     if (p->smem < (size_t)3 * 2 * 4096) p->smem = (size_t)3 * 2 * 4096;
     return 7209;
 }
@@ -1009,6 +1011,8 @@
 
 template <typename T> constexpr int wgrad_fold_waves = (WgradCfg<T>::WK - 1) * WgradCfg<T>::WCO * WgradCfg<T>::WCI;
 
+static bool wgrad_tile_s2(const WgradArgs& a, int esz) { return esz == 2 && a.ks == 3 && a.stride == 2; }
+
 int wgrad_select(const WgradArgs& a0, int dtype, const WgradBn& bn, WgradPlan* p) {
     *p = WgradPlan{};
     p->a = a0;
@@ -1034,7 +1038,7 @@
         PW = ((1 << a.lTW) - 1) * lstride + a.ks; PH = ((1 << a.lTH) - 1) * lstride + a.ks;
         NPIX = a.TN * PH * PW;
         need = (NPIX * 8 + NW * 64 - 1) / (NW * 64);
-        smem = ((size_t)(1 << lBM) + NPIX) * 192;
+        smem = ((size_t)(1 << lBM) + NPIX) * lds_layout::TR_ROW_B;
         if (need <= M2 && smem <= 150 * 1024) break;
     }
     a.n_groups = (a.ipe + a.TN - 1) / a.TN;
@@ -1060,6 +1064,7 @@
     p->maxv = need <= M1 ? M1 : M2;
     p->grid = dim3(p->nsplit * tiles, 1, p->E); p->block = dim3(NW * 64);
     const size_t fold = (size_t)(esz == 2 ? wgrad_fold_waves<bf16> : wgrad_fold_waves<float>) * (p->taps == 9 ? 3 : 1) * 4096;
+    if (wgrad_tile_s2(a, esz)) smem = (size_t)(1 << lBM) * lds_layout::TR_ROW_B + (size_t)NPIX * lds_layout::TR_ROW_B_S2;
     p->smem = smem < fold ? fold : smem;
     return p->code = 6000 + p->taps * 100 + p->maxv;
 }
@@ -1072,6 +1077,10 @@
 
 template <typename T> static int wgrad_tile_launch(const WgradPlan& p, hipStream_t st) {
     constexpr int M1 = 48 / WgradCfg<T>::NW, M2 = 80 / WgradCfg<T>::NW;
+    if constexpr (sizeof(T) == 2) {
+        if (wgrad_tile_s2(p.a, p.esz))
+            return p.maxv == M1 ? wgrad_go<conv_wgrad_kernel<T, 9, M1, true>>(p, st) : wgrad_go<conv_wgrad_kernel<T, 9, M2, true>>(p, st);
+    }
     if (p.maxv == M1) return p.taps == 9 ? wgrad_go<conv_wgrad_kernel<T, 9, M1>>(p, st) : wgrad_go<conv_wgrad_kernel<T, 1, M1>>(p, st);
     return p.taps == 9 ? wgrad_go<conv_wgrad_kernel<T, 9, M2>>(p, st) : wgrad_go<conv_wgrad_kernel<T, 1, M2>>(p, st);
 }
diff --git a/pmoe_amd/csrc/lds_layout.h b/pmoe_amd/csrc/lds_layout.h
--- /dev/null
+++ b/pmoe_amd/csrc/lds_layout.h
@@ -0,0 +1,25 @@
+#pragma once
+
+namespace lds_layout {
+
+constexpr int ROW_B = 128;
+
+constexpr int key_row(int row) { return (row >> 1) & 7; }
+
+template <bool MF16> constexpr int key_col(int col) { return MF16 ? (col & 6) : ((col >> 1) & 7); }
+
+constexpr int key_col_s2(int col) { return ((col & 1) << 2) | ((col >> 1) & 3); }
+
+constexpr int row_chunk_off(int row, int chunk, int key) { return row * ROW_B + ((chunk ^ key) << 4); }
+constexpr int dma_src_chunk_off(int jj, int key) { return (jj ^ key) << 4; }
+constexpr int frag_chunk_mf32(int ks, int lane) { return ks * 2 + (lane >> 5); }
+constexpr int frag_chunk_mf16(int ks, int lane) { return ks * 4 + (lane >> 4); }
+
+constexpr int TR_ROW_B = 192;
+constexpr int TR_ROW_B_S2 = 160;
+template <bool S2> constexpr int tr_row_b() { return S2 ? TR_ROW_B_S2 : TR_ROW_B; }
+template <bool S2> constexpr int tr_off(int pix, int cbyte) { return pix * tr_row_b<S2>() + cbyte; }
+constexpr int tr_lane_cbyte(int sub, int lane) { return (sub * 32 + 16 * ((lane >> 4) & 1) + 4 * (lane & 3)) * 2; }
+constexpr int tr_lane_pixel(int tt, int lane) { return 8 * (lane >> 5) + 4 * tt + ((lane >> 2) & 3); }
+
+}
```

Result: slower. 1871 samples/s (-1.0%).
